# sangminwoo/Temporal-Span-Proposal-Network-VidVRD

Measured on AMD Instinct MI355X. Metric: tracklet-pairs/sec scored (N=32, T=150, D=2048), higher is better.
Workload: dtype f32

## Files before the change

include/tspn_mi355x.h:

```cpp
#ifndef TSPN_MI355X_H
#define TSPN_MI355X_H

#include <stddef.h>
#include <stdint.h>

#ifdef __cplusplus
extern "C" {
#endif

#define TSPN_ABI_VERSION 7

enum {
  TSPN_OK = 0,
  TSPN_EINVAL = -1,
  TSPN_EUNSUPPORTED = -2,
  TSPN_EWORKSPACE = -3,
  TSPN_ELAUNCH = -4,
  TSPN_EDEVICE = -5
};

#define TSPN_STATUS_WORDS 16
enum {
  TSPN_STATUS_FAULT = 0,
  TSPN_STATUS_FAULT_INFO = 1,
  TSPN_STATUS_CONV_ERR = 2,
  TSPN_STATUS_CONV_CHECKS = 3
};
enum {
  TSPN_FAULT_HANDOVER = 1
};
int tspn_status_attach(int32_t* host_words);
int tspn_status_fault(void);
int tspn_status_clear(void);
int tspn_status_selftest(int32_t* reached_end, void* stream);

#define TSPN_GEOM_CHANNELS 8

enum {
  TSPN_CONV_DIRECT = 0,
  TSPN_CONV_WINOGRAD63 = 1,
  TSPN_CONV_WINOGRAD63_F16X3 = 2
};

int tspn_version(void);
size_t tspn_fused_desc_size(void);
size_t tspn_fused_bf16_desc_size(void);
const char* tspn_last_error(void);
const char* tspn_error_string(int code);

size_t tspn_predicate_head_workspace_bytes(int64_t P, int64_t F, int64_t K);
int tspn_predicate_head_f32(const float* x, int64_t P, int64_t F, int64_t ldx,
                            const float* W, const float* b, int64_t K,
                            float* out, int apply_sigmoid,
                            void* workspace, size_t workspace_bytes, void* stream);

size_t tspn_predicate_head_norm_workspace_bytes(int64_t P, int64_t F, int64_t K, int64_t first,
                                                int64_t block, int64_t nblocks);
int tspn_predicate_head_norm_f32(const float* x, int64_t P, int64_t F, int64_t ldx,
                                 const float* W, const float* b, int64_t K,
                                 int64_t first, int64_t block, int64_t nblocks,
                                 float* out, int apply_sigmoid,
                                 void* workspace, size_t workspace_bytes, void* stream);

int tspn_feature_preprocess_f32(float* feats, int64_t P, int64_t F, int64_t ld,
                                int64_t first, int64_t block, int64_t nblocks,
                                void* stream);

int tspn_proposal_pair_filter_i64(const int64_t* pairs, const int64_t* pair_off,
                                  const int64_t* trackid, const int64_t* track_off, int64_t S,
                                  int64_t* out_idx, int64_t* out_count, int64_t* out_num_tracks,
                                  void* stream);
int tspn_gather_rows_f32(const float* src, int64_t ld, int64_t F, const int64_t* idx,
                         int64_t idx_base, int64_t R, float* out, void* stream);

int tspn_ppn_pair_matrix_topk_f32(const float* cls, int64_t B, int64_t N, int64_t Cin,
                                  int64_t H, int64_t Cout,
                                  const float* ws1, const float* bs1,
                                  const float* ws2, const float* bs2,
                                  const float* wo1, const float* bo1,
                                  const float* wo2, const float* bo2,
                                  int64_t topk, float* out_mat, int64_t* out_idx,
                                  void* stream);

int tspn_traj_iou_f32(const float* boxes1, int64_t N1, const float* boxes2, int64_t N2,
                      int64_t B, int64_t T, float* out, void* stream);

int tspn_traj_iou_tail_f64(const double* a, const int32_t* len_a, const double* b, int64_t U, int64_t N,
                           int64_t L, float* out, void* stream);

int tspn_pair_index_i64(int64_t N, int64_t base, int64_t* pairs, void* stream);

int tspn_pair_gather_f32(const float* feats, const float* boxes, int64_t NT, int64_t T,
                         int64_t D, const int64_t* pairs, int64_t P,
                         float* out_feat, float* out_geom, void* stream);

int tspn_pack_conv3_f32(const float* W, int64_t M, int64_t Cin, int64_t split,
                        float* packed, void* stream);

int tspn_conv3_f32(const float* x, int64_t B, int64_t Cin, int64_t T,
                   const float* packed, int64_t M, const float* bias, int relu,
                   float* y, void* stream);

int tspn_conv3_tc_f32(const float* x, int64_t B, int64_t T, int64_t Cin,
                      const float* packed, int64_t M, const float* bias, int relu,
                      float* y, void* stream);

int tspn_pack_conv3_wino63_frag_f32(const float* W, int64_t M, int64_t Cin, int64_t split, float* frag,
                                    void* stream);
size_t tspn_conv3_tc_wino63_workspace_bytes(int64_t B, int64_t T, int64_t Cin);
int tspn_conv3_tc_wino63_f32(const float* x, int64_t B, int64_t T, int64_t Cin, const float* frag,
                             int64_t M, const float* bias, int relu, float* y,
                             void* workspace, size_t workspace_bytes, void* stream);
int tspn_conv3_tc_wino63_set_piece_form(int form);

size_t tspn_pack_conv3_wino63_f16x3_elements(int64_t M, int64_t Cin, int64_t split);
int tspn_pack_conv3_wino63_f16x3(const float* W, int64_t M, int64_t Cin, int64_t split, int16_t* packed, void* stream);
size_t tspn_conv3_tc_wino63_f16x3_workspace_bytes(int64_t B, int64_t T, int64_t Cin, int64_t M);
int tspn_conv3_tc_wino63_f16x3(const float* x, int64_t B, int64_t T, int64_t Cin, const int16_t* packed,
                               int64_t M, const float* bias, int relu, float* y,
                               void* workspace, size_t workspace_bytes, void* stream);
int tspn_conv3_tc_wino63_f16x3_set_tail_split(int on);


int tspn_heads_f32(int mode, const float* a, const float* b, int64_t lda,
                   const int64_t* ia, const int64_t* ib, int64_t idx_stride, const float* bias,
                   const float* Wh, const float* bh, int64_t H,
                   int64_t P, int64_t C, int64_t T, float* out, void* stream);

int tspn_heads_pairgrid_f32(const float* y, int64_t B, int64_t N, int64_t C, int64_t T,
                            const float* Wh, const float* bh, int64_t H, float* out,
                            void* stream);

size_t tspn_heads_pairgrid_f16x3_split_bytes(int64_t C, int64_t H);
int tspn_heads_pairgrid_f16x3_set_force_exact(int on);
int tspn_heads_pairgrid_f16x3(const float* y, int64_t ldt, int64_t B, int64_t N, int64_t C, int64_t T,
                              const float* Wh, const float* bh, int64_t H, void* split_buf, size_t split_bytes,
                              float* out, void* stream);

int tspn_temporal_mean_f32(const float* x, int64_t R, int64_t T, int64_t Cdim,
                           int layout_tc, float* out, void* stream);
int tspn_temporal_sum_f32(const float* x, int64_t R, int64_t T, int64_t Cdim, float* out, void* stream);

int tspn_pair_rows_f32(const float* src, int64_t NT, int64_t D, const int64_t* pairs,
                       int64_t P, float* out, void* stream);

int tspn_transpose_td_f32(const float* x, int64_t R, int64_t T, int64_t D, float* out,
                          void* stream);

size_t tspn_decode_topk_workspace_bytes(int64_t S, int64_t P, int64_t topk_pair);
int tspn_decode_topk_f32(const float* rel_logit, const int64_t* pairs,
                         const float* cls_sub, const float* cls_obj, int64_t ld,
                         int64_t seg_rows, int64_t row_mul, int64_t S, int64_t P, int64_t K,
                         int64_t NO, int64_t topk_pair, int64_t topk_seg,
                         float* out_score, int64_t* out_triplet, int64_t* out_pair_tid,
                         void* workspace, size_t workspace_bytes, void* stream);

int tspn_decode_spans_f32(const float* heads, int64_t P, int64_t A, int64_t T,
                          const float* sizes_host, int64_t top_k, double nms_threshold,
                          int64_t pre_nms, int64_t* out_anchor, int64_t* out_span,
                          float* out_span_f, float* out_score, int64_t* out_count, void* stream);

typedef struct tspn_fused_desc {
  int64_t B, N, T, D;
  int64_t A, K;
  const float* feats;
  const int64_t* pairs;
  int64_t P;
  int64_t canonical_pairs;
  const float* conv_packed;
  int64_t conv_algo;
  const float* conv_bias;
  const float* head_w;
  const float* head_b;
  const float* cls_w;
  const float* cls_b;
  float* out_heads;
  float* out_logits;
  void* workspace;
  size_t workspace_bytes;
  void* ev_conv_begin;
  void* ev_conv_end;
  void* ev_logits_ready;
  const float* conv_weight;
  int64_t conv_check;
} tspn_fused_desc;

size_t tspn_forward_fused_workspace_bytes(const tspn_fused_desc* d);
int tspn_forward_fused_f32(const tspn_fused_desc* d, void* stream);

#define TSPN_CONV_CHECK_HOT_SLOTS 64
#define TSPN_CONV_CHECK_HOT_OFFSET 256
#define TSPN_CONV_CHECK_SCRATCH_BYTES (TSPN_CONV_CHECK_HOT_OFFSET + 256 * TSPN_CONV_CHECK_HOT_SLOTS)
int tspn_conv3_spot_check_f32(const float* x, int64_t B, int64_t T, int64_t Cin, const float* W, int64_t M,
                              int64_t Cw, int64_t split, const float* bias, int relu, const float* y, int64_t ldy,
                              uint64_t* scratch, int64_t rows, void* stream);

size_t tspn_span_predicate_workspace_bytes(int64_t NT, int64_t T, int64_t D, int64_t K);
int tspn_span_predicate_f32(const float* feats, int64_t NT, int64_t T, int64_t D, const int64_t* pairs,
                            const int64_t* spans, int64_t P, const float* cls_w, const float* cls_b,
                            int64_t K, float* out, void* workspace, size_t workspace_bytes, void* stream);

size_t tspn_decode_span_relations_workspace_bytes(int64_t S, int64_t N, int64_t T, int64_t D, int64_t P, int64_t J,
                                                  int64_t K, int64_t topk_per_span);
int tspn_decode_span_relations_f32(const float* feats, int64_t S, int64_t N, int64_t T, int64_t D,
                                   const int64_t* pairs, int64_t P, const int64_t* spans, const float* span_scores,
                                   const int64_t* span_counts, int64_t J, const float* cls_w, const float* cls_b,
                                   int64_t K, const float* cls_logits, int64_t NO, int64_t topk_per_span,
                                   int64_t topk_per_seg, float* out_score, int64_t* out_triplet,
                                   int64_t* out_pair_tid, int64_t* out_span, int64_t* out_span_rank,
                                   int64_t* out_valid, void* workspace, size_t workspace_bytes, void* stream);

int tspn_cast_bf16(const float* src, int64_t n, uint16_t* dst, void* stream);
int tspn_pack_conv3_bf16(const float* W, int64_t M, int64_t Cin, int64_t split, uint16_t* packed,
                         void* stream);
int tspn_pack_heads_bf16(const float* W, int64_t H, int64_t C, uint16_t* packed, void* stream);
int tspn_conv3_tc_bf16(const uint16_t* x, int64_t B, int64_t T, int64_t Cin, const uint16_t* packed,
                       int64_t M, const float* bias, float* y, int64_t ldm, void* stream);
int tspn_heads_pairgrid_bf16(const float* y, int64_t ldm, int64_t B, int64_t N, int64_t C, int64_t T,
                             const uint16_t* head_packed, const float* head_b, int64_t H, float* out,
                             void* stream);
int tspn_temporal_mean_bf16(const uint16_t* x, int64_t R, int64_t T, int64_t D, float* out, void* stream);

typedef struct tspn_fused_bf16_desc {
  int64_t B, N, T, D;
  int64_t A, K;
  const uint16_t* feats;
  const int64_t* pairs;
  int64_t P;
  const uint16_t* conv_packed;
  const float* conv_bias;
  const uint16_t* head_packed;
  const float* head_b;
  const float* cls_w;
  const float* cls_b;
  float* out_heads;
  float* out_logits;
  void* workspace;
  size_t workspace_bytes;
  void* ev_conv_begin;
  void* ev_conv_end;
  void* ev_logits_ready;
} tspn_fused_bf16_desc;

size_t tspn_forward_fused_bf16_workspace_bytes(const tspn_fused_bf16_desc* d);
int tspn_forward_fused_bf16(const tspn_fused_bf16_desc* d, void* stream);

int tspn_pair_plan_i32(const int64_t* pairs, int64_t P, int64_t B, int64_t N, int32_t* s_list, int32_t* o_list,
                       int32_t* counts, int32_t* head, int32_t* next, int32_t* rank_ws, void* stream);
size_t tspn_heads_pairlist_bf16_workspace_bytes(int64_t B, int64_t N, int64_t P);
int tspn_heads_pairlist_bf16(const float* y, int64_t ldm, int64_t B, int64_t N, int64_t C, int64_t T,
                             const int64_t* pairs, int64_t P, const uint16_t* head_packed, const float* head_b,
                             int64_t H, float* out, void* workspace, size_t workspace_bytes, void* stream);
size_t tspn_forward_fused_bf16_pairs_workspace_bytes(const tspn_fused_bf16_desc* d);
int tspn_forward_fused_bf16_pairs(const tspn_fused_bf16_desc* d, void* stream);

int tspn_pack_span_cls_bf16(const float* cls_w, int64_t K, int64_t D, uint16_t* packed, void* stream);
size_t tspn_span_predicate_bf16_workspace_bytes(int64_t NT, int64_t T, int64_t D, int64_t K, int64_t P);
int tspn_span_predicate_bf16(const uint16_t* feats, int64_t NT, int64_t T, int64_t D, const int64_t* pairs,
                             const int64_t* spans, int64_t P, const uint16_t* cls_packed, const float* cls_b,
                             int64_t K, float* out, void* workspace, size_t workspace_bytes, void* stream);
size_t tspn_decode_span_relations_bf16_workspace_bytes(int64_t S, int64_t N, int64_t T, int64_t D, int64_t P, int64_t J,
                                                       int64_t K, int64_t topk_per_span);
int tspn_decode_span_relations_bf16(const uint16_t* feats, int64_t S, int64_t N, int64_t T, int64_t D,
                                    const int64_t* pairs, int64_t P, const int64_t* spans, const float* span_scores,
                                    const int64_t* span_counts, int64_t J, const uint16_t* cls_packed,
                                    const float* cls_b, int64_t K, const float* cls_logits, int64_t NO,
                                    int64_t topk_per_span, int64_t topk_per_seg, float* out_score, int64_t* out_triplet,
                                    int64_t* out_pair_tid, int64_t* out_span, int64_t* out_span_rank,
                                    int64_t* out_valid, void* workspace, size_t workspace_bytes, void* stream);

int tspn_temporal_encoder_heads_f32(const float* x, int64_t P, int64_t C, int64_t T,
                                    const float* conv_packed, const float* conv_bias,
                                    const float* head_w, const float* head_b, int64_t H,
                                    float* h_ws, float* out_heads, void* stream);
// ... 112 lines not shown
```

temporal-span-proposal-network-vidvrd_amd/_abi.py:

```python
import ctypes
import os
import re
import threading

HERE = os.path.dirname(os.path.abspath(__file__))
ROOT = os.path.dirname(HERE)
LIB_PATH = os.environ.get("TSPN_LIB_PATH") or os.path.join(HERE, "libtspn_mi355x.so")
HEADER_PATH = os.path.join(ROOT, "include", "tspn_mi355x.h")

ABI_VERSION = 7
TSPN_OK = 0
TSPN_EINVAL = -1
TSPN_EUNSUPPORTED = -2
TSPN_EWORKSPACE = -3
TSPN_ELAUNCH = -4
TSPN_EDEVICE = -5
STATUS_WORDS = 16
STATUS_FAULT, STATUS_FAULT_INFO, STATUS_CONV_ERR, STATUS_CONV_CHECKS = 0, 1, 2, 3
FAULT_HANDOVER = 1
CONV_CHECK_HOT_OFFSET, CONV_CHECK_SCRATCH_BYTES = 256, 256 + 256 * 64
GEOM_CHANNELS = 8
CONV_DIRECT, CONV_WINOGRAD63, CONV_WINOGRAD63_F16X3 = 0, 1, 2

_c_f32p = ctypes.c_void_p
_c_i64p = ctypes.c_void_p
_i64 = ctypes.c_int64
_int = ctypes.c_int
_vp = ctypes.c_void_p
_sz = ctypes.c_size_t


class FusedDesc(ctypes.Structure):
    _fields_ = [
        ("B", _i64), ("N", _i64), ("T", _i64), ("D", _i64),
        ("A", _i64), ("K", _i64),
        ("feats", _vp), ("pairs", _vp), ("P", _i64), ("canonical_pairs", _i64),
        ("conv_packed", _vp), ("conv_algo", _i64), ("conv_bias", _vp),
        ("head_w", _vp), ("head_b", _vp),
        ("cls_w", _vp), ("cls_b", _vp),
        ("out_heads", _vp), ("out_logits", _vp),
        ("workspace", _vp), ("workspace_bytes", _sz),
        ("ev_conv_begin", _vp), ("ev_conv_end", _vp), ("ev_logits_ready", _vp),
        ("conv_weight", _vp), ("conv_check", _i64),
    ]


class FusedBf16Desc(ctypes.Structure):
    _fields_ = [
        ("B", _i64), ("N", _i64), ("T", _i64), ("D", _i64),
        ("A", _i64), ("K", _i64),
        ("feats", _vp), ("pairs", _vp), ("P", _i64),
        ("conv_packed", _vp), ("conv_bias", _vp),
        ("head_packed", _vp), ("head_b", _vp),
        ("cls_w", _vp), ("cls_b", _vp),
        ("out_heads", _vp), ("out_logits", _vp),
        ("workspace", _vp), ("workspace_bytes", _sz),
        ("ev_conv_begin", _vp), ("ev_conv_end", _vp), ("ev_logits_ready", _vp),
    ]


PROTOTYPES = {
    "tspn_version": (_int, []),
    "tspn_fused_desc_size": (_sz, []),
    "tspn_fused_bf16_desc_size": (_sz, []),
    "tspn_last_error": (ctypes.c_char_p, []),
    "tspn_error_string": (ctypes.c_char_p, [_int]),
    "tspn_status_attach": (_int, [_vp]),
    "tspn_status_fault": (_int, []),
    "tspn_status_clear": (_int, []),
    "tspn_status_selftest": (_int, [_vp, _vp]),
    "tspn_conv3_spot_check_f32": (_int, [_vp, _i64, _i64, _i64, _vp, _i64, _i64, _i64, _vp, _int, _vp, _i64, _vp, _i64, _vp]),
    "tspn_predicate_head_workspace_bytes": (_sz, [_i64, _i64, _i64]),
    "tspn_predicate_head_f32": (_int, [_vp, _i64, _i64, _i64, _vp, _vp, _i64, _vp, _int, _vp, _sz, _vp]),
    "tspn_predicate_head_norm_workspace_bytes": (_sz, [_i64, _i64, _i64, _i64, _i64, _i64]),
    "tspn_predicate_head_norm_f32": (_int, [_vp, _i64, _i64, _i64, _vp, _vp, _i64, _i64, _i64, _i64, _vp, _int,
                                            _vp, _sz, _vp]),
    "tspn_feature_preprocess_f32": (_int, [_vp, _i64, _i64, _i64, _i64, _i64, _i64, _vp]),
    "tspn_proposal_pair_filter_i64": (_int, [_vp, _vp, _vp, _vp, _i64, _vp, _vp, _vp, _vp]),
    "tspn_gather_rows_f32": (_int, [_vp, _i64, _i64, _vp, _i64, _i64, _vp, _vp]),
    "tspn_ppn_pair_matrix_topk_f32": (_int, [_vp, _i64, _i64, _i64, _i64, _i64,
                                             _vp, _vp, _vp, _vp, _vp, _vp, _vp, _vp,
                                             _i64, _vp, _vp, _vp]),
    "tspn_traj_iou_f32": (_int, [_vp, _i64, _vp, _i64, _i64, _i64, _vp, _vp]),
    "tspn_traj_iou_tail_f64": (_int, [_vp, _vp, _vp, _i64, _i64, _i64, _vp, _vp]),
    "tspn_pair_index_i64": (_int, [_i64, _i64, _vp, _vp]),
    "tspn_pair_gather_f32": (_int, [_vp, _vp, _i64, _i64, _i64, _vp, _i64, _vp, _vp, _vp]),
    "tspn_pack_conv3_f32": (_int, [_vp, _i64, _i64, _i64, _vp, _vp]),
    "tspn_conv3_f32": (_int, [_vp, _i64, _i64, _i64, _vp, _i64, _vp, _int, _vp, _vp]),
    "tspn_conv3_tc_f32": (_int, [_vp, _i64, _i64, _i64, _vp, _i64, _vp, _int, _vp, _vp]),
    "tspn_heads_f32": (_int, [_int, _vp, _vp, _i64, _vp, _vp, _i64, _vp, _vp, _vp, _i64, _i64, _i64,
                              _i64, _vp, _vp]),
    "tspn_heads_pairgrid_f32": (_int, [_vp, _i64, _i64, _i64, _i64, _vp, _vp, _i64, _vp, _vp]),
    "tspn_heads_pairgrid_f16x3_split_bytes": (_sz, [_i64, _i64]),
    "tspn_heads_pairgrid_f16x3_set_force_exact": (_int, [_int]),
    "tspn_heads_pairgrid_f16x3": (_int, [_vp, _i64, _i64, _i64, _i64, _i64, _vp, _vp, _i64, _vp, _sz, _vp, _vp]),
    "tspn_temporal_mean_f32": (_int, [_vp, _i64, _i64, _i64, _int, _vp, _vp]),
    "tspn_temporal_sum_f32": (_int, [_vp, _i64, _i64, _i64, _vp, _vp]),
    "tspn_pair_rows_f32": (_int, [_vp, _i64, _i64, _vp, _i64, _vp, _vp]),
    "tspn_transpose_td_f32": (_int, [_vp, _i64, _i64, _i64, _vp, _vp]),
    "tspn_decode_topk_workspace_bytes": (_sz, [_i64, _i64, _i64]),
    "tspn_decode_topk_f32": (_int, [_vp, _vp, _vp, _vp, _i64, _i64, _i64, _i64, _i64, _i64, _i64, _i64, _i64,
                                    _vp, _vp, _vp, _vp, _sz, _vp]),
    "tspn_decode_spans_f32": (_int, [_vp, _i64, _i64, _i64, ctypes.POINTER(ctypes.c_float), _i64,
                                     ctypes.c_double, _i64, _vp, _vp, _vp, _vp, _vp, _vp]),
    "tspn_forward_fused_workspace_bytes": (_sz, [ctypes.POINTER(FusedDesc)]),
    "tspn_forward_fused_f32": (_int, [ctypes.POINTER(FusedDesc), _vp]),
    "tspn_temporal_encoder_heads_f32": (_int, [_vp, _i64, _i64, _i64, _vp, _vp, _vp, _vp, _i64,
                                               _vp, _vp, _vp]),
    "tspn_pack_conv2d_f32": (_int, [_vp, _i64, _i64, _i64, _i64, _vp, _vp]),
    "tspn_conv2d_nhwc_f32": (_int, [_vp, _i64, _i64, _i64, _i64, _vp, _i64, _i64, _i64, _i64, _i64, _vp, _vp,
                                    _int, _vp, _vp]),
    "tspn_pack_conv2d_frag_f32": (_int, [_vp, _i64, _i64, _i64, _i64, _vp, _vp]),
    "tspn_conv2d_nhwc_frag_f32": (_int, [_vp, _i64, _i64, _i64, _i64, _vp, _i64, _i64, _i64, _i64, _i64, _vp, _vp,
                                         _int, _vp, _vp]),
    "tspn_pack_conv2d_frag_bf16": (_int, [_vp, _i64, _i64, _i64, _i64, _vp, _vp]),
    "tspn_conv2d_nhwc_bf16": (_int, [_vp, _i64, _i64, _i64, _i64, _vp, _i64, _i64, _i64, _i64, _i64, _vp, _vp,
                                     _int, _vp, _vp]),
    "tspn_roi_align_nhwc_f32": (_int, [_vp, _i64, _i64, _i64, _i64, _vp, _i64, _i64, ctypes.c_float, _int, _int,
                                       _int, _vp, _vp]),
    "tspn_pack_conv2d_frag_cin4_f32": (_int, [_vp, _i64, _i64, _i64, _i64, _vp, _vp]),
    "tspn_conv2d_nhwc_cin4_f32": (_int, [_vp, _i64, _i64, _i64, _vp, _i64, _i64, _i64, _i64, _i64, _vp, _int, _vp, _vp]),
    "tspn_max_pool_nhwc_f32": (_int, [_vp, _i64, _i64, _i64, _i64, _i64, _i64, _i64, _vp, _int, _vp]),
    "tspn_bottleneck_tail_bf16": (_int, [_vp, _i64, _i64, _i64, _i64, _vp, _vp, _vp, _vp, _vp, _vp, _vp]),
    "tspn_bottleneck_block_bf16": (_int, [_vp, _i64, _i64, _i64, _i64, _vp, _vp, _vp, _vp, _vp, _vp, _vp, _vp]),
    "tspn_bottleneck_block_proj_bf16": (_int, [_vp, _i64, _i64, _i64, _i64, _i64, _i64, _vp, _vp, _vp, _vp, _vp, _vp, _vp, _vp,
                                               _vp, _vp]),
    "tspn_bottleneck_block_res_bf16": (_int, [_vp, _i64, _i64, _i64, _i64, _i64, _i64, _vp, _vp, _vp, _vp, _vp, _vp, _vp, _vp, _vp]),
    "tspn_bottleneck_tail_io_bf16": (_int, [_vp, _i64, _i64, _i64, _i64, _vp, _vp, _vp, _vp, _vp, _vp, _vp]),
    "tspn_bottleneck_tail_pipe_bf16": (_int, [_vp, _i64, _i64, _i64, _i64, _vp, _vp, _vp, _vp, _vp, _vp, _i64, _vp]),
    "tspn_bottleneck_tail_next_bf16": (_int, [_vp, _i64, _i64, _i64, _i64, _vp, _vp, _vp, _vp, _vp, _vp, _vp, _vp, _vp, _vp]),
    "tspn_stem_bf16_workspace_bytes": (_sz, [_i64, _i64, _i64]),
    "tspn_pack_stem_bf16": (_int, [_vp, _i64, _vp, _vp]),
    "tspn_stem_conv_bf16": (_int, [_vp, _i64, _i64, _i64, _vp, _i64, _vp, _vp, _sz, _vp, _vp]),
    "tspn_max_pool_nhwc_bf16": (_int, [_vp, _i64, _i64, _i64, _i64, _i64, _i64, _i64, _vp, _vp]),
    "tspn_stem_pool_bf16": (_int, [_vp, _i64, _i64, _i64, _vp, _i64, _vp, _vp, _sz, _vp, _vp]),
    "tspn_roi_align_nhwc_bf16": (_int, [_vp, _i64, _i64, _i64, _i64, _vp, _i64, _i64, ctypes.c_float, _int, _int,
                                        _int, _vp, _vp]),
    "tspn_roi_align_nhwc_f32_bf16out": (_int, [_vp, _i64, _i64, _i64, _i64, _vp, _i64, _i64, ctypes.c_float, _int, _int,
                                               _int, _vp, _vp]),
    "tspn_pack_conv3_wino63_frag_f32": (_int, [_vp, _i64, _i64, _i64, _vp, _vp]),
    "tspn_conv3_tc_wino63_workspace_bytes": (_sz, [_i64, _i64, _i64]),
    "tspn_conv3_tc_wino63_f32": (_int, [_vp, _i64, _i64, _i64, _vp, _i64, _vp, _int, _vp, _vp, _sz, _vp]),
    "tspn_conv3_tc_wino63_set_piece_form": (_int, [_int]),
    "tspn_pack_conv3_wino63_f16x3_elements": (_sz, [_i64, _i64, _i64]),
    "tspn_pack_conv3_wino63_f16x3": (_int, [_vp, _i64, _i64, _i64, _vp, _vp]),
    "tspn_conv3_tc_wino63_f16x3_workspace_bytes": (_sz, [_i64, _i64, _i64, _i64]),
    "tspn_conv3_tc_wino63_f16x3": (_int, [_vp, _i64, _i64, _i64, _vp, _i64, _vp, _int, _vp, _vp, _sz, _vp]),
    "tspn_conv3_tc_wino63_f16x3_set_tail_split": (_int, [_int]),
    "tspn_span_predicate_workspace_bytes": (_sz, [_i64, _i64, _i64, _i64]),
    "tspn_span_predicate_f32": (_int, [_vp, _i64, _i64, _i64, _vp, _vp, _i64, _vp, _vp, _i64, _vp, _vp, _sz, _vp]),
    "tspn_decode_span_relations_workspace_bytes": (_sz, [_i64] * 8),
    "tspn_decode_span_relations_f32": (_int, [_vp, _i64, _i64, _i64, _i64, _vp, _i64, _vp, _vp, _vp, _i64, _vp, _vp, _i64,
                                              _vp, _i64, _i64, _i64, _vp, _vp, _vp, _vp, _vp, _vp, _vp, _sz, _vp]),
    "tspn_cast_bf16": (_int, [_vp, _i64, _vp, _vp]),
    "tspn_pack_conv3_bf16": (_int, [_vp, _i64, _i64, _i64, _vp, _vp]),
    "tspn_transpose_cast_bf16": (_int, [_vp, _i64, _i64, _i64, _vp, _vp]),
    "tspn_heads_dense_bf16": (_int, [_vp, _i64, _i64, _i64, _i64, _vp, _vp, _i64, _vp, _vp]),
    "tspn_temporal_encoder_heads_bf16": (_int, [_vp, _i64, _i64, _i64, _vp, _vp, _vp, _vp, _i64, _vp, _vp, _vp]),
    "tspn_pack_heads_bf16": (_int, [_vp, _i64, _i64, _vp, _vp]),
    "tspn_conv3_tc_bf16": (_int, [_vp, _i64, _i64, _i64, _vp, _i64, _vp, _vp, _i64, _vp]),
    "tspn_heads_pairgrid_bf16": (_int, [_vp, _i64, _i64, _i64, _i64, _i64, _vp, _vp, _i64, _vp, _vp]),
    "tspn_temporal_mean_bf16": (_int, [_vp, _i64, _i64, _i64, _vp, _vp]),
    "tspn_forward_fused_bf16_workspace_bytes": (_sz, [ctypes.POINTER(FusedBf16Desc)]),
    "tspn_forward_fused_bf16": (_int, [ctypes.POINTER(FusedBf16Desc), _vp]),
    "tspn_pair_plan_i32": (_int, [_vp, _i64, _i64, _i64, _vp, _vp, _vp, _vp, _vp, _vp, _vp]),
    "tspn_heads_pairlist_bf16_workspace_bytes": (_sz, [_i64, _i64, _i64]),
    "tspn_heads_pairlist_bf16": (_int, [_vp, _i64, _i64, _i64, _i64, _i64, _vp, _i64, _vp, _vp, _i64, _vp, _vp, _sz, _vp]),
    "tspn_forward_fused_bf16_pairs_workspace_bytes": (_sz, [ctypes.POINTER(FusedBf16Desc)]),
    "tspn_forward_fused_bf16_pairs": (_int, [ctypes.POINTER(FusedBf16Desc), _vp]),
    "tspn_pack_span_cls_bf16": (_int, [_vp, _i64, _i64, _vp, _vp]),
    "tspn_span_predicate_bf16_workspace_bytes": (_sz, [_i64] * 5),
    "tspn_span_predicate_bf16": (_int, [_vp, _i64, _i64, _i64, _vp, _vp, _i64, _vp, _vp, _i64, _vp, _vp, _sz, _vp]),
    "tspn_decode_span_relations_bf16_workspace_bytes": (_sz, [_i64] * 8),
    "tspn_decode_span_relations_bf16": (_int, [_vp, _i64, _i64, _i64, _i64, _vp, _i64, _vp, _vp, _vp, _i64, _vp, _vp, _i64,
                                               _vp, _i64, _i64, _i64, _vp, _vp, _vp, _vp, _vp, _vp, _vp, _sz, _vp]),
    "tspn_span_anchor_labels": (_int, [_vp, ctypes.POINTER(ctypes.c_float), _i64, _i64, _i64, _i64, ctypes.c_double,
                                      ctypes.c_double, _vp, _vp, _vp]),
    "tspn_span_loss_f32": (_int, [_vp, _vp, ctypes.POINTER(ctypes.c_float), _vp, _vp, _vp, _i64, _i64, _i64, _i64,
                                 ctypes.c_double, _vp, _vp, _vp]),
    "tspn_span_loss_finish": (_int, [_vp, _i64, _i64, _i64, _vp, _vp, _vp]),
    "tspn_span_anchor_sample_partials": (_i64, [_i64]),
    "tspn_span_anchor_sample": (_int, [_vp, _i64, ctypes.c_uint64, _int, _i64, _i64, _vp, _vp, _vp, _vp]),
    "tspn_pair_labels_f32": (_int, [_vp] * 9 + [_i64] * 6 + [ctypes.c_double, _int, _vp, _vp, _vp, _vp, _vp]),
    "tspn_eval_traj_volume_f64": (_int, [_vp, _vp, _i64, _vp, _vp]),
    "tspn_eval_viou_f64": (_int, [_vp, _vp, _vp, _vp, _vp, _i64, _vp, _vp, _vp]),
    "tspn_eval_greedy_match_f64": (_int, [_vp, _vp, _i64, _i64, ctypes.c_double, _vp, _vp, _vp, _vp]),
}

_lib = None
_lock = threading.Lock()


def header_symbols(path=HEADER_PATH):
    text = open(path).read()
    text = re.sub(r"/\*.*?\*/", "", text, flags=re.S)
    return sorted(set(re.findall(r"\b(tspn_[a-z0-9_]+)\s*\(", text)))


def lib():
    global _lib
    if _lib is not None:
        return _lib
    with _lock:
        if _lib is not None:
            return _lib
        if not os.path.exists(LIB_PATH):
            raise RuntimeError(
                f"TSPN HIP library not built: {LIB_PATH} is missing. Run "
                "`python -c 'import __graft_entry__ as g; g.build()'` (needs hipcc). "
                "There is no CPU fallback.")
        handle = ctypes.CDLL(LIB_PATH)
        for name, (res, args) in PROTOTYPES.items():
            try:
                fn = getattr(handle, name)
            except AttributeError as exc:
                raise RuntimeError(f"TSPN HIP library {LIB_PATH} does not export {name}") from exc
            fn.restype = res
            fn.argtypes = args
        if handle.tspn_version() != ABI_VERSION:
            raise RuntimeError(f"TSPN ABI version mismatch: library {LIB_PATH} reports "
                               f"{handle.tspn_version()}, host expects {ABI_VERSION} (stale build? run "
                               "__graft_entry__.build())")
        for fn, struct in (("tspn_fused_desc_size", FusedDesc), ("tspn_fused_bf16_desc_size", FusedBf16Desc)):
            if getattr(handle, fn)() != ctypes.sizeof(struct):
                raise RuntimeError(f"TSPN ABI mismatch: {fn}() = {getattr(handle, fn)()} but the host binding "
                                   f"has {ctypes.sizeof(struct)} bytes (stale {LIB_PATH}?)")
        _lib = handle
    return _lib


class TspnError(RuntimeError):
    def __init__(self, code, message):
        super().__init__(f"tspn error {code}: {message}")
        self.code = code


def check(rc):
    if rc != TSPN_OK:
        l = lib()
        msg = l.tspn_last_error().decode("utf-8", "replace")
        if not msg:
            msg = l.tspn_error_string(rc).decode()
        raise TspnError(rc, msg)
```

temporal-span-proposal-network-vidvrd_amd/build.py:

```python
import glob
import json
import os
import re
import shutil
import subprocess
import sys

HERE = os.path.dirname(os.path.abspath(__file__))
ROOT = os.path.dirname(HERE)
CSRC = os.path.join(HERE, "csrc")
CSRC_EVAL = os.path.join(CSRC, "eval")
CSRC_REL = os.path.join(CSRC, "relations")
CSRC_PAIRLIST = os.path.join(CSRC, "pairlist")
CSRC_SPANBF16 = os.path.join(CSRC, "spanbf16")
CSRC_PAIRF16 = os.path.join(CSRC, "pairf16")
CSRC_SPANLOSS = os.path.join(CSRC, "spanloss")
CSRC_SPANSAMPLE = os.path.join(CSRC, "spansample")
CSRC_PAIRLABELS = os.path.join(CSRC, "pairlabels")
LIB_NAME = "libtspn_mi355x.so"
LIB_PATH = os.path.join(HERE, LIB_NAME)
ARCH = "gfx950"

FLAGS = [
    f"--offload-arch={ARCH}", "-O3", "-std=c++17", "-fPIC",
    "-ffp-contract=off",
    "-fno-gpu-rdc", "-Wall", "-Wno-unused-function",
    "-Rpass-analysis=kernel-resource-usage",
    f"-I{os.path.join(ROOT, 'include')}", f"-I{CSRC}",
]
OBJ_DIR = os.path.join(HERE, "build", "obj")
RES_PATH = os.path.join(HERE, "kernel_resources.json")

NO_SPILL_KERNELS = ("conv3_wino63_kernel", "heads_pairgrid4_kernel", "heads_pairgrid3_kernel",
                    "conv2d_nhwc_frag_kernel", "conv2d_nhwc_bf16_kernel", "conv2d_nhwc_cin4_kernel",
                    "bottleneck_bf16_kernel", "bottleneck_pipe_bf16_kernel", "conv3_bf16_big_kernel", "heads_pairgrid_bf16_kernel",
                    "heads_pairlist_bf16_kernel", "heads_pair_f16x3_kernel",
                    "tail_io_bf16_kernel", "bottleneck_block_bf16_kernel")


def sources():
    return sorted(glob.glob(os.path.join(CSRC, "*.hip")) + glob.glob(os.path.join(CSRC_EVAL, "*.hip")) +
                  glob.glob(os.path.join(CSRC_REL, "*.hip")) + glob.glob(os.path.join(CSRC_PAIRLIST, "*.hip")) +
                  glob.glob(os.path.join(CSRC_SPANBF16, "*.hip")) + glob.glob(os.path.join(CSRC_SPANLOSS, "*.hip")) +
                  glob.glob(os.path.join(CSRC_PAIRF16, "*.hip")) + glob.glob(os.path.join(CSRC_SPANSAMPLE, "*.hip")) +
                  glob.glob(os.path.join(CSRC_PAIRLABELS, "*.hip")))


def _headers():
    return glob.glob(os.path.join(CSRC, "*.h")) + glob.glob(os.path.join(CSRC_EVAL, "*.h")) + \
        glob.glob(os.path.join(CSRC_REL, "*.h")) + glob.glob(os.path.join(CSRC_PAIRLIST, "*.h")) + \
        glob.glob(os.path.join(CSRC_SPANBF16, "*.h")) + glob.glob(os.path.join(CSRC_SPANLOSS, "*.h")) + \
        glob.glob(os.path.join(CSRC_PAIRF16, "*.h")) + glob.glob(os.path.join(CSRC_SPANSAMPLE, "*.h")) + \
        glob.glob(os.path.join(CSRC_PAIRLABELS, "*.h")) + \
        glob.glob(os.path.join(ROOT, "include", "*.h")) + \
        [os.path.abspath(__file__)]


def needs_build():
    if not os.path.exists(LIB_PATH) or not os.path.exists(RES_PATH):
        return True
    t = os.path.getmtime(LIB_PATH)
    return any(os.path.getmtime(d) > t for d in sources() + _headers())


def _obj_of(src):
    return os.path.join(OBJ_DIR, os.path.basename(src)[:-4] + ".o")


_REMARK = re.compile(r"remark:\s+(Function Name|TotalSGPRs|VGPRs|AGPRs|ScratchSize \[bytes/lane\]|Occupancy \[waves/SIMD\]|"
                     r"SGPRs Spill|VGPRs Spill|LDS Size \[bytes/block\]): (\S+)")
_KEYS = {"TotalSGPRs": "sgprs", "VGPRs": "vgprs", "AGPRs": "agprs", "ScratchSize [bytes/lane]": "scratch_bytes",
         "Occupancy [waves/SIMD]": "occupancy", "SGPRs Spill": "sgpr_spill", "VGPRs Spill": "vgpr_spill",
         "LDS Size [bytes/block]": "lds_bytes"}


def _demangle(names):
    filt = shutil.which("llvm-cxxfilt") or shutil.which("c++filt")
    if not names or not filt:
        return list(names)
    out = subprocess.run([filt], input="\n".join(names), stdout=subprocess.PIPE, text=True).stdout.split("\n")
    return out[:len(names)]


def _parse_resources(log):
    res, cur, kept, skip = {}, None, [], 0
    for line in log.split("\n"):
        m = _REMARK.search(line)
        if m:
            if m.group(1) == "Function Name":
                cur = res.setdefault(m.group(2), {})
            elif cur is not None:
                cur[_KEYS[m.group(1)]] = int(m.group(2))
            skip = 2
            continue
        if "remark:" in line and "kernel-resource-usage" in line:
            skip = 2
            continue
        if skip and (line.lstrip().startswith("|") or re.match(r"\s*\d+ \|", line)):
            skip -= 1
            continue
        skip = 0
        kept.append(line)
    names = list(res)
    return dict(zip(_demangle(names), (res[n] for n in names))), "\n".join(kept)


def _compile_one(hipcc, src, verbose):
    cmd = [hipcc] + FLAGS + ["-c", src, "-o", _obj_of(src)]
    if verbose:
        print("[tspn build]", " ".join(cmd), flush=True)
    res = subprocess.run(cmd, cwd=CSRC, stdout=subprocess.PIPE, stderr=subprocess.STDOUT, text=True)
    resources, log = _parse_resources(res.stdout)
    if res.returncode == 0:
        with open(_obj_of(src) + ".res.json", "w") as fh:
            json.dump(resources, fh, indent=1, sort_keys=True)
    return src, res.returncode, log


def kernel_resources():
    with open(RES_PATH) as fh:
        return json.load(fh)


def check_no_spill(resources):
    bad = []
    for name, r in resources.items():
        if any(k in name for k in NO_SPILL_KERNELS) and (r.get("sgpr_spill", 0) or r.get("vgpr_spill", 0)
                                                          or r.get("scratch_bytes", 0)):
            bad.append(f"{name}: {r}")
    return bad


def build(force=False, verbose=True, jobs=None):
    if not force and not needs_build():
        return LIB_PATH
    hipcc = shutil.which("hipcc") or "/opt/rocm/bin/hipcc"
    if not os.path.exists(hipcc):
        raise RuntimeError("hipcc not found: cannot build the TSPN HIP library")
    os.makedirs(OBJ_DIR, exist_ok=True)
    newest_header = max(os.path.getmtime(h) for h in _headers())
    stale = [s for s in sources()
             if force or not os.path.exists(_obj_of(s)) or not os.path.exists(_obj_of(s) + ".res.json")
             or os.path.getmtime(_obj_of(s)) < max(os.path.getmtime(s), newest_header)]
    from concurrent.futures import ThreadPoolExecutor
    jobs = jobs or min(len(stale) or 1, os.cpu_count() or 1, 8)
    with ThreadPoolExecutor(max_workers=jobs) as pool:
        results = list(pool.map(lambda s: _compile_one(hipcc, s, verbose), stale))
    for src, rc, log in results:
        if log.strip() and (verbose or rc):
            print(log, flush=True)
        if rc:
            raise RuntimeError(f"hipcc failed on {src} (exit {rc})")
    wanted = {_obj_of(s) for s in sources()}
    for o in glob.glob(os.path.join(OBJ_DIR, "*.o")):
        if o not in wanted:
            os.remove(o)
            if os.path.exists(o + ".res.json"):
                os.remove(o + ".res.json")
    resources = {}
    for o in sorted(wanted):
        with open(o + ".res.json") as fh:
            resources.update(json.load(fh))
    bad = check_no_spill(resources)
    if bad:
        raise RuntimeError("kernels with split asm load / wait sequences must not spill:\n  " + "\n  ".join(bad))
    with open(RES_PATH, "w") as fh:
        json.dump(resources, fh, indent=1, sort_keys=True)
    tmp = LIB_PATH + ".tmp"
    cmd = [hipcc, f"--offload-arch={ARCH}", "-shared", "-fPIC", "-fno-gpu-rdc"] + sorted(wanted) + ["-o", tmp]
    if verbose:
        print("[tspn build]", " ".join(cmd), flush=True)
    subprocess.run(cmd, check=True, cwd=CSRC)
    os.replace(tmp, LIB_PATH)
    return LIB_PATH


if __name__ == "__main__":
    build(force="--force" in sys.argv)
    print(LIB_PATH)
```

temporal-span-proposal-network-vidvrd_amd/csrc/pairf16/tspn_heads_pair_f16x3.hip:

```cpp
#include "tspn_common.h"
#include "tspn_device.h"

namespace {
using namespace tspn_dev;

constexpr int PF_S = 8, PF_O = 8, PF_T = 32, PF_CK = 32;
constexpr int PF_ROWS = PF_S + PF_O;
constexpr int PF_STAGE = PF_ROWS * PF_CK * PF_T;
constexpr int PF_THREADS = 64 * PF_S;
constexpr size_t PF_SMEM = sizeof(float) * 2 * PF_STAGE;
constexpr int PF_HDR_BYTES = 256;
constexpr int PF_KSTEP_BYTES = 2 * 64 * 16;
constexpr float PF_LO = 2048.f, PF_LO_INV = 1.f / 2048.f;
constexpr float PF_RANGE = 16384.f;

typedef _Float16 f16x2 __attribute__((ext_vector_type(2)));

std::atomic<int> g_force_exact{0};

__device__ __forceinline__ unsigned split_lo(unsigned h2, float as0, float as1) {
  unsigned d;
  const float neg = -PF_LO;
  asm("v_fma_mixlo_f16 %0, %1, %2, %3 op_sel_hi:[1,0,0]" : "=v"(d) : "v"(h2), "s"(neg), "v"(as0));
  asm("v_fma_mixhi_f16 %0, %1, %2, %3 op_sel:[1,0,0] op_sel_hi:[1,0,0]" : "+v"(d) : "v"(h2), "s"(neg), "v"(as1));
  return d;
}

__global__ __launch_bounds__(1024) void pairf16_scale_kernel(const float* __restrict__ Wh, int C, int H,
                                                            unsigned* __restrict__ hdr) {
  __shared__ unsigned bad_s[16];
  const int lane = threadIdx.x & 63, h = threadIdx.x >> 6;
  float mx = 0.f;
  bool finite = true;
  if (h < H) {
    for (int c = lane; c < C; c += 64) {
      const float a = fabsf(Wh[(int64_t)h * C + c]);
      finite = finite && (a < __builtin_inff());
      mx = fmaxf(mx, a);
    }
  }
#pragma unroll
  for (int o = 32; o > 0; o >>= 1) mx = fmaxf(mx, __shfl_xor(mx, o, 64));
  const bool all_finite = __all(finite);
  int e = 0;
  (void)frexpf(mx, &e);
  const bool bad = h < H && (!all_finite || !(mx >= 0x1p-100f) || e > 100);
  if (lane == 0) {
    bad_s[h] = bad ? 1u : 0u;
    hdr[1 + h] = __float_as_uint((h < H && !bad) ? ldexpf(1.f, e) : 1.f);
  }
  __syncthreads();
  if (threadIdx.x == 0) {
    unsigned f = 0;
    for (int i = 0; i < 16; ++i) f |= bad_s[i];
    hdr[0] = f;
  }
  if (threadIdx.x >= 17 && threadIdx.x < PF_HDR_BYTES / 4) hdr[threadIdx.x] = 0;
}

__global__ __launch_bounds__(64) void pairf16_pack_kernel(const float* __restrict__ Wh, int C, int H,
                                                         const unsigned* __restrict__ hdr, u32x4* __restrict__ frag) {
  const int lane = threadIdx.x, h = lane & 15, kg = lane >> 4;
  const float scale = 1.f / __uint_as_float(hdr[1 + h]);
  unsigned hi[4], lo[4];
#pragma unroll
  for (int ip = 0; ip < 4; ++ip) {
    f16x2 wh, wl;
#pragma unroll
    for (int e = 0; e < 2; ++e) {
      const int c = blockIdx.x * PF_CK + kg + 4 * (2 * ip + e);
      const float w = (h < H) ? Wh[(int64_t)h * C + c] * scale : 0.f;
      const _Float16 a = (_Float16)w;
      wh[e] = a;
      wl[e] = (_Float16)((w - (float)a) * PF_LO);
    }
    hi[ip] = __builtin_bit_cast(unsigned, wh);
    lo[ip] = __builtin_bit_cast(unsigned, wl);
  }
  frag[(int64_t)blockIdx.x * 128 + lane] = u32x4{hi[0], hi[1], hi[2], hi[3]};
  frag[(int64_t)blockIdx.x * 128 + 64 + lane] = u32x4{lo[0], lo[1], lo[2], lo[3]};
}

__device__ __noinline__ void exact_tile(const float* __restrict__ y, int64_t ldt, int C, int T, int N, int H,
                                        const float* __restrict__ Wh, const float* __restrict__ bh,
                                        float* __restrict__ out, int64_t b, int sb, int ob, int t0) {
  const int t = t0 + (threadIdx.x & 31);
  if (t >= T) return;
  for (int idx = threadIdx.x >> 5; idx < PF_S * PF_O * H; idx += PF_THREADS / 32) {
    const int pair = idx / H, h = idx - pair * H;
    const int s = sb * PF_S + (pair >> 3), o = ob * PF_O + (pair & 7);
    if (s >= N || o >= N || s == o) continue;
    const float* up = y + ((b * N + s) * 2 * (int64_t)C) * ldt + t;
    const float* vp = y + ((b * N + o) * 2 * (int64_t)C + C) * ldt + t;
    const float* w = Wh + (int64_t)h * C;
    float sum = 0.f;
    for (int c = 0; c < C; ++c) sum = __builtin_fmaf(w[c], tspn::relu_f32(up[c * ldt] + vp[c * ldt]), sum);
    const int64_t p = b * N * (int64_t)(N - 1) + (int64_t)s * (N - 1) + o - (o > s ? 1 : 0);
    out[(p * H + h) * (int64_t)T + t] = sum + (bh ? bh[h] : 0.f);
  }
}

__global__ __launch_bounds__(PF_THREADS, 1) void heads_pair_f16x3_kernel(
    const float* __restrict__ y, int64_t ldt, int C, int T, int N, int H, const float* __restrict__ Wh,
    const float* __restrict__ bh, const unsigned* __restrict__ hdr, const u32x4* __restrict__ frag,
    float* __restrict__ out, int ntb, int nob, int nsb, int64_t ngroups, int force_exact) {
  extern __shared__ __attribute__((aligned(16))) char smem_raw[];
  float* S = reinterpret_cast<float*>(smem_raw);

  const int tid = threadIdx.x;
  const int lane = tid & 63;
  const int wave = __builtin_amdgcn_readfirstlane(tid >> 6);
  const int j = lane & 15, kg = lane >> 4;
  int sb, ob;
  const int64_t G = pair_stage_group(blockIdx.x, nsb, nob, sb, ob);
  if (G >= ngroups) return;
  const int64_t b = G / ntb;
  const int t0 = (int)(G - b * ntb) * PF_T;
  const int64_t rowlen = 2 * (int64_t)C * ldt;

  if (force_exact | (int)hdr[0]) {
    exact_tile(y, ldt, C, T, N, H, Wh, bh, out, b, sb, ob, t0);
    return;
  }

  const __amdgpu_buffer_rsrc_t rsrc_y = buffer_rsrc(y + b * N * rowlen, (int)(unsigned)((int64_t)N * rowlen * 4));
  unsigned voff[2];
  const unsigned loff = (unsigned)((lane >> 3) * ldt + min((int64_t)t0 + (lane & 7) * 4, ldt - 4));
#pragma unroll
  for (int r = 0; r < 2; ++r) {
    const int row = 2 * wave + r;
    const int local = row < PF_S ? sb * PF_S + row : ob * PF_O + (row - PF_S);
    const int64_t trk = min(local, N - 1);
    voff[r] = (unsigned)((trk * rowlen + (row < PF_S ? 0 : (int64_t)C * ldt) + loff) * 4);
  }
  const int piece_bytes = (int)(8 * ldt * 4);
  int y_soff = 0;
  auto stage = [&](int buf) {
#pragma unroll
    for (int r = 0; r < 2; ++r) {
#pragma unroll
      for (int q = 0; q < 4; ++q)
        bglds16(rsrc_y, voff[r], y_soff + q * piece_bytes, S + buf * PF_STAGE + ((2 * wave + r) * PF_CK + 8 * q) * PF_T);
    }
    y_soff += 4 * piece_bytes;
  };

  f32x4 acc_hi[PF_O][2], acc_lo[PF_O][2];
#pragma unroll
  for (int o = 0; o < PF_O; ++o) {
#pragma unroll
    for (int cb = 0; cb < 2; ++cb) acc_hi[o][cb] = acc_lo[o][cb] = f32x4{0.f, 0.f, 0.f, 0.f};
  }

  const int nk = C / PF_CK;
  stage(0);
  u32x4 wh = frag[lane], wl = frag[64 + lane];
  asm volatile("s_waitcnt vmcnt(0)" ::: "memory");
  __syncthreads();
  const float* urow = S + (wave * PF_CK + kg) * PF_T + 2 * j;
  const float* vrow = S + (PF_S * PF_CK + kg) * PF_T + 2 * j;
  const float* trow = vrow + wave * PF_CK * PF_T;
  float mu = 0.f, mv = 0.f;
  for (int k = 0; k < nk; ++k) {
    const int buf = k & 1;
    u32x4 whn = wh, wln = wl;
    if (k + 1 < nk) {
      stage(buf ^ 1);
      whn = frag[(int64_t)(k + 1) * 128 + lane];
      wln = frag[(int64_t)(k + 1) * 128 + 64 + lane];
    }
    const float* ub = urow + buf * PF_STAGE;
    const float* vb = vrow + buf * PF_STAGE;
    const float* tb = trow + buf * PF_STAGE;
    f32x2 u[8];
#pragma unroll
    for (int i = 0; i < 8; ++i) {
      u[i] = *reinterpret_cast<const f32x2*>(ub + 4 * i * PF_T);
      const f32x2 vt = *reinterpret_cast<const f32x2*>(tb + 4 * i * PF_T);
      mu = __builtin_elementwise_maximum(__builtin_elementwise_maximum(mu, __builtin_fabsf(u[i][0])), __builtin_fabsf(u[i][1]));
      mv = __builtin_elementwise_maximum(__builtin_elementwise_maximum(mv, __builtin_fabsf(vt[0])), __builtin_fabsf(vt[1]));
    }
    const f16x8 a_hi = __builtin_bit_cast(f16x8, wh), a_lo = __builtin_bit_cast(f16x8, wl);
    f32x2 v[8], vn[8];
    u32x4 fh[2], fl[2], gh[2], gl[2];
#pragma unroll
    for (int i = 0; i < 8; ++i) v[i] = *reinterpret_cast<const f32x2*>(vb + 4 * i * PF_T);
#pragma unroll
    for (int o = 0; o <= PF_O; ++o) {
      if (o + 1 < PF_O) {
#pragma unroll
        for (int i = 0; i < 8; ++i) vn[i] = *reinterpret_cast<const f32x2*>(vb + ((o + 1) * PF_CK + 4 * i) * PF_T);
      }
// ... 148 lines not shown
```

temporal-span-proposal-network-vidvrd_amd/csrc/tspn_common.h:

```cpp
#pragma once
#include <hip/hip_runtime.h>

#include <atomic>
#include <cstdarg>
#include <cstdint>
#include <cstdio>
#include <initializer_list>

#include "tspn_mi355x.h"

namespace tspn {

char* err_buf();
constexpr int kErrBufLen = 512;

inline int fail(int code, const char* fmt, ...) {
  va_list ap;
  va_start(ap, fmt);
  vsnprintf(err_buf(), kErrBufLen, fmt, ap);
  va_end(ap);
  return code;
}

int status_check(const char* what);

inline int check_launch(const char* what) {
  hipError_t e = hipGetLastError();
  if (e != hipSuccess) return fail(TSPN_ELAUNCH, "%s: %s", what, hipGetErrorString(e));
  return status_check(what);
}

inline int64_t ceil_div(int64_t a, int64_t b) { return (a + b - 1) / b; }
inline bool aligned16(const void* p) { return (reinterpret_cast<uintptr_t>(p) & 15) == 0; }
template <class... P>
inline bool all_aligned16(const P*... p) {
  return (aligned16(p) && ...);
}
__host__ __device__ inline int64_t next_pow2(int64_t n) {
  int64_t p = 1;
  while (p < n) p <<= 1;
  return p;
}

__device__ __forceinline__ float relu_f32(float v) { return __builtin_elementwise_maximum(v, 0.f); }
__device__ __forceinline__ float maximum_f32(float a, float b) { return __builtin_elementwise_maximum(a, b); }

__device__ __forceinline__ unsigned order_key(float v) {
  if (v != v) return 0xffffffffu;
  const unsigned u = __float_as_uint(v + 0.f);
  return (u & 0x80000000u) ? ~u : (u | 0x80000000u);
}

__device__ __forceinline__ bool key_before(unsigned ka, int ia, unsigned kb, int ib) {
  return ka > kb || (ka == kb && ia < ib);
}

__device__ __forceinline__ unsigned long long wave_max_u64(unsigned long long v) {
#pragma unroll
  for (int o = 32; o > 0; o >>= 1) {
    const unsigned long long other = __shfl_xor(v, o, 64);
    v = other > v ? other : v;
  }
  return v;
}

struct LdsLimit {
  static constexpr int kMaxDevices = 64;
  std::atomic<size_t> set[kMaxDevices] = {};
  int ensure(const void* fn, size_t bytes, const char* what) {
    int dev = -1;
    (void)hipGetDevice(&dev);
    const bool tracked = dev >= 0 && dev < kMaxDevices;
    if (tracked && set[dev].load(std::memory_order_relaxed) >= bytes) return TSPN_OK;
    hipError_t e = hipFuncSetAttribute(fn, hipFuncAttributeMaxDynamicSharedMemorySize, (int)bytes);
    if (e != hipSuccess)
      return fail(TSPN_ELAUNCH, "%s: hipFuncSetAttribute(%zu bytes of LDS): %s", what, bytes,
                  hipGetErrorString(e));
    if (tracked) set[dev].store(bytes, std::memory_order_relaxed);
    return TSPN_OK;
  }
};

int conv3_tc_direct(const float* x, int64_t B, int64_t T, int64_t Cin, const float* packed, int64_t M,
                    const float* bias, int relu, float* y, int64_t ldy, void* stream);
bool wino63_supported(int64_t Cin, int64_t M);
size_t wino63_workspace_bytes(int64_t B, int64_t T, int64_t Cin);
int wino63_input_transform(const float* x, int64_t B, int64_t T, int64_t Cin, void* workspace,
                           size_t workspace_bytes, void* stream, uint64_t* hot = nullptr);
int wino63_contract(const void* workspace, int64_t B, int64_t T, int64_t Cin, const float* frag, int64_t M,
                    const float* bias, int relu, float* y, int64_t ldy, void* stream);
int conv3_tc_wino63(const float* x, int64_t B, int64_t T, int64_t Cin, const float* frag, int64_t M,
                    const float* bias, int relu, float* y, int64_t ldy, void* workspace,
                    size_t workspace_bytes, void* stream);
bool wino63_f16x3_supported(int64_t Cin, int64_t M);
size_t wino63_f16x3_workspace_bytes(int64_t B, int64_t T, int64_t Cin, int64_t M);
int wino63_f16x3_input_transform(const float* x, int64_t B, int64_t T, int64_t Cin, int64_t M, void* workspace,
                                 size_t workspace_bytes, void* stream, uint64_t* hot = nullptr);
int wino63_f16x3_contract(void* workspace, size_t workspace_bytes, int64_t B, int64_t T, int64_t Cin,
                          const int16_t* packed, int64_t M, const float* bias, int relu, float* y, int64_t ldy,
                          void* stream);
int heads_pairgrid(const float* y, int64_t ldt, int64_t B, int64_t N, int64_t C, int64_t T,
                   const float* Wh, const float* bh, int64_t H, float* out, void* stream, float* Wp12 = nullptr);
size_t heads_pair_f16x3_split_bytes(int64_t C, int64_t H);
bool heads_pair_f16x3_supported(const float* y, int64_t ldt, int64_t N, int64_t C, int64_t T, int64_t H, const float* out);
int heads_pair_f16x3(const float* y, int64_t ldt, int64_t B, int64_t N, int64_t C, int64_t T, const float* Wh,
                     const float* bh, int64_t H, void* split_buf, size_t split_bytes, float* out, void* stream);
inline size_t align_up(size_t a, size_t b) { return (a + b - 1) / b * b; }
int linear(const float* x, int64_t P, int64_t F, int64_t ldx, const float* W, int64_t ldw,
           const float* b, int64_t K, float* out, int apply_sigmoid, void* workspace,
           size_t workspace_bytes, void* stream);
size_t pair_predicate_workspace_bytes(int64_t NT, int64_t D, int64_t K);
int pair_predicate(const float* fbar, int64_t NT, int64_t D, const int64_t* pairs, int64_t P,
                   const float* cls_w, const float* cls_b, int64_t K, float* out, void* workspace,
                   size_t workspace_bytes, void* stream);
size_t span_prefix_workspace_bytes(int64_t NT, int64_t T, int64_t D, int64_t K);
int span_prefix_stage(const float* feats, int64_t NT, int64_t T, int64_t D, const float* cls_w, int64_t K,
                      void* workspace, size_t workspace_bytes, void* stream, const float** G_out,
                      const double** PS_out, const char* who);
inline size_t span_cand_bytes(int64_t S, int64_t P, int64_t J, int64_t R) {
  return align_up((size_t)S * P * J * R * sizeof(float), 256);
}
int segment_span_topk(const unsigned* key, const float* sc, const int* ix, const int64_t* pairs, const int64_t* spans,
                      const int64_t* span_counts, const float* cls_logits, int64_t S, int64_t N, int64_t NO, int64_t P,
                      int64_t J, int64_t R, int64_t topk_per_seg, float* out_score, int64_t* out_triplet,
                      int64_t* out_pair_tid, int64_t* out_span, int64_t* out_span_rank, int64_t* out_valid, void* stream,
                      const char* what);
int span_relation_sizes(const char* who, int64_t S, int64_t N, int64_t T, int64_t D, int64_t P, int64_t J, int64_t K,
                        int64_t NO, int64_t topk_per_span, int64_t topk_per_seg);
int span_relation_limits(const char* who, int64_t P, int64_t J, int64_t K, int64_t topk_per_span, int64_t topk_per_seg,
                         int64_t* R);

}

#define TSPN_REQUIRE(cond, code, ...)                 \
  do {                                                \
    if (!(cond)) return tspn::fail(code, __VA_ARGS__); \
  } while (0)

#define TSPN_STREAM(s) reinterpret_cast<hipStream_t>(s)

namespace tspn {

inline int tail_shape_checks(const char* what, int64_t NB, int64_t H, int64_t W, int64_t CM, bool channels_ok,
                             const char* channel_rule) {
  TSPN_REQUIRE(NB >= 0 && H > 0 && W > 0, TSPN_EINVAL, "%s: bad sizes", what);
  TSPN_REQUIRE(channels_ok, TSPN_EUNSUPPORTED, "%s: %s (got %lld)", what, channel_rule, (long long)CM);
  return TSPN_OK;
}
inline int operand_checks(const char* what, std::initializer_list<const void*> operands, bool alias_free = true,
                          const char* alias_rule = nullptr) {
  bool all = true, aligned = true;
  for (const void* p : operands) {
    all = all && p != nullptr;
    aligned = aligned && aligned16(p);
  }
  TSPN_REQUIRE(all, TSPN_EINVAL, "%s: null pointer", what);
  TSPN_REQUIRE(alias_free, TSPN_EINVAL, "%s: %s", what, alias_rule);
  TSPN_REQUIRE(aligned, TSPN_EUNSUPPORTED, "%s: operands must be 16-byte aligned", what);
  return TSPN_OK;
}
inline int tail_operand_checks(const char* what, int64_t H, int64_t W, std::initializer_list<const void*> operands) {
  if (int rc = operand_checks(what, operands)) return rc;
  TSPN_REQUIRE(H < (1 << 20) && W < (1 << 20), TSPN_EUNSUPPORTED, "%s: dimension too large", what);
  return TSPN_OK;
}

inline int window_shape_checks(const char* what, bool sizes_ok, bool window_ok, const char* window_rule, int64_t H,
                               int64_t W, int64_t KH, int64_t KW, int64_t stride, int64_t pad, int64_t* OH, int64_t* OW) {
  TSPN_REQUIRE(sizes_ok, TSPN_EINVAL, "%s: bad sizes", what);
  TSPN_REQUIRE(window_ok, TSPN_EUNSUPPORTED, "%s: %s", what, window_rule);
  TSPN_REQUIRE(H + 2 * pad >= KH && W + 2 * pad >= KW, TSPN_EINVAL, "%s: empty output", what);
  *OH = (H + 2 * pad - KH) / stride + 1, *OW = (W + 2 * pad - KW) / stride + 1;
  return TSPN_OK;
}
inline int conv_operand_checks(const char* what, const void* x, const void* w, const void* out, const void* bias,
                               const void* residual, bool channels_ok, const char* channel_rule, int64_t H, int64_t W,
                               int64_t Cin, int64_t Cout) {
  TSPN_REQUIRE(x && w && out, TSPN_EINVAL, "%s: null pointer", what);
  TSPN_REQUIRE(channels_ok, TSPN_EUNSUPPORTED, "%s: needs %s (Cin=%lld Cout=%lld)", what, channel_rule, (long long)Cin,
               (long long)Cout);
  TSPN_REQUIRE(all_aligned16(x, w, out, bias, residual), TSPN_EUNSUPPORTED, "%s: operands must be 16-byte aligned", what);
  TSPN_REQUIRE(H < (1 << 20) && W < (1 << 20) && Cin < (1 << 24) && Cout < (1 << 24), TSPN_EUNSUPPORTED,
               "%s: dimension too large", what);
  return TSPN_OK;
}

}
```

temporal-span-proposal-network-vidvrd_amd/csrc/tspn_fused.hip:

```cpp
#include <algorithm>

#include "tspn_common.h"

namespace {

struct FusedLayout {
  size_t xt, y, bias2, fbar, pooled, lin, vt, hwp, hot, psplit, total;
  size_t vt_bytes;
  size_t psplit_bytes;
  size_t lin_bytes;
};

FusedLayout layout_of(const tspn_fused_desc* d) {
  FusedLayout L{};
  const size_t NT = (size_t)d->B * d->N, T = d->T, D = d->D, C = 2 * D;
  size_t off = 0;
  auto take = [&](size_t bytes) {
    const size_t o = off;
    off += tspn::align_up(bytes, 256);
    return o;
  };
  L.xt = take(NT * D * T * sizeof(float));
  L.y = take(NT * 2 * C * tspn::align_up(T, 4) * sizeof(float));
  L.bias2 = take(2 * C * sizeof(float));
  L.fbar = take(NT * D * sizeof(float));
  L.pooled = take(256);
  L.lin_bytes = tspn::pair_predicate_workspace_bytes((int64_t)NT, (int64_t)D, d->K);
  L.lin = take(L.lin_bytes);
  L.vt_bytes = (D % 32 == 0) ? tspn::wino63_workspace_bytes((int64_t)NT, (int64_t)T, (int64_t)D) : 0;
  if (d->conv_algo == TSPN_CONV_WINOGRAD63_F16X3)
    L.vt_bytes = tspn::wino63_f16x3_workspace_bytes((int64_t)NT, (int64_t)T, (int64_t)D, (int64_t)(2 * C));
  L.vt = take(L.vt_bytes);
  L.hwp = take(C * 12 * sizeof(float));
  L.psplit_bytes = (d->conv_algo == TSPN_CONV_WINOGRAD63_F16X3 && 3 * d->A == 12)
                       ? tspn::heads_pair_f16x3_split_bytes((int64_t)C, 12) : 0;
  L.psplit = take(L.psplit_bytes);
  L.hot = take(TSPN_CONV_CHECK_SCRATCH_BYTES);
  L.total = off;
  return L;
}

int check_desc(const tspn_fused_desc* d) {
  TSPN_REQUIRE(d != nullptr, TSPN_EINVAL, "tspn_forward_fused: null descriptor");
  TSPN_REQUIRE(d->B >= 0 && d->N >= 0 && d->T > 0 && d->D > 0 && d->A > 0 && d->K > 0 &&
                   d->P >= 0,
               TSPN_EINVAL, "tspn_forward_fused: bad sizes B=%lld N=%lld T=%lld D=%lld A=%lld K=%lld P=%lld",
               (long long)d->B, (long long)d->N, (long long)d->T, (long long)d->D, (long long)d->A,
               (long long)d->K, (long long)d->P);
  TSPN_REQUIRE(3 * d->A <= 16, TSPN_EUNSUPPORTED, "tspn_forward_fused: 3*A=%lld > 16",
               (long long)(3 * d->A));
  return TSPN_OK;
}

}

extern "C" size_t tspn_forward_fused_workspace_bytes(const tspn_fused_desc* d) {
  if (check_desc(d) != TSPN_OK) return 0;
  return layout_of(d).total;
}

extern "C" int tspn_forward_fused_f32(const tspn_fused_desc* d, void* stream) {
  int rc = check_desc(d);
  if (rc) return rc;
  if (d->P == 0 || d->B * d->N == 0) return TSPN_OK;
  TSPN_REQUIRE(d->feats && d->pairs && d->conv_packed && d->conv_bias && d->head_w && d->head_b &&
                   d->cls_w && d->cls_b && d->out_heads && d->out_logits,
               TSPN_EINVAL, "tspn_forward_fused: null pointer in descriptor");
  const FusedLayout L = layout_of(d);
  TSPN_REQUIRE(d->workspace && d->workspace_bytes >= L.total, TSPN_EWORKSPACE,
               "tspn_forward_fused: workspace %zu < %zu bytes", d->workspace_bytes, L.total);
  TSPN_REQUIRE((reinterpret_cast<uintptr_t>(d->workspace) & 255) == 0, TSPN_EINVAL,
               "tspn_forward_fused: workspace must be 256-byte aligned");
  char* ws = static_cast<char*>(d->workspace);
  float* xt = reinterpret_cast<float*>(ws + L.xt);
  float* y = reinterpret_cast<float*>(ws + L.y);
  float* bias2 = reinterpret_cast<float*>(ws + L.bias2);
  float* fbar = reinterpret_cast<float*>(ws + L.fbar);
  float* pooled = reinterpret_cast<float*>(ws + L.pooled);
  void* lin = ws + L.lin;
  const int64_t NT = d->B * d->N, T = d->T, D = d->D, C = 2 * D, H = 3 * d->A;
  hipStream_t s = TSPN_STREAM(stream);

  const bool tc = (D % 16 == 0) && tspn::all_aligned16(d->feats, d->conv_packed);
  TSPN_REQUIRE(d->conv_algo == TSPN_CONV_DIRECT || d->conv_algo == TSPN_CONV_WINOGRAD63 ||
                   d->conv_algo == TSPN_CONV_WINOGRAD63_F16X3,
               TSPN_EINVAL,
               "tspn_forward_fused: conv_algo must be TSPN_CONV_DIRECT (0), TSPN_CONV_WINOGRAD63 (1) or "
               "TSPN_CONV_WINOGRAD63_F16X3 (2), got %d",
               (int)d->conv_algo);
  const bool f16x3 = d->conv_algo == TSPN_CONV_WINOGRAD63_F16X3;
  const bool w63 = d->conv_algo == TSPN_CONV_WINOGRAD63 || f16x3;
  TSPN_REQUIRE(!w63 || (tc && tspn::wino63_supported(D, 2 * C)), TSPN_EUNSUPPORTED,
               "tspn_forward_fused: TSPN_CONV_WINOGRAD63 needs D %% 32 == 0 and 16-byte aligned operands "
               "(pack the weights with tspn_pack_conv3_f32 and pass TSPN_CONV_DIRECT otherwise)");
  TSPN_REQUIRE(!f16x3 || tspn::wino63_f16x3_supported(D, 2 * C), TSPN_EUNSUPPORTED,
               "tspn_forward_fused: TSPN_CONV_WINOGRAD63_F16X3 needs D %% 64 == 0 (4D %% 256 == 0)");

  hipError_t e = hipMemsetAsync(bias2 + C, 0, C * sizeof(float), s);
  if (e == hipSuccess)
    e = hipMemcpyAsync(bias2, d->conv_bias, C * sizeof(float), hipMemcpyDeviceToDevice, s);
  if (e != hipSuccess)
    return tspn::fail(TSPN_ELAUNCH, "tspn_forward_fused: bias staging: %s", hipGetErrorString(e));

  if ((rc = tspn_temporal_mean_f32(d->feats, NT, T, D, 1, fbar, stream))) return rc;
  (void)pooled;
  if ((rc = tspn::pair_predicate(fbar, NT, D, d->pairs, d->P, d->cls_w, d->cls_b, d->K, d->out_logits, lin,
                                 L.lin_bytes, stream)))
    return rc;
  if (d->ev_logits_ready) (void)hipEventRecord(static_cast<hipEvent_t>(d->ev_logits_ready), s);

  const int64_t ldy =
      (tc && d->canonical_pairs && T % 2 == 0) ? (int64_t)tspn::align_up((size_t)T, 4) : T;
  if (!tc && (rc = tspn_transpose_td_f32(d->feats, NT, T, D, xt, stream))) return rc;
  const bool guard = w63 && d->conv_check > 0 && d->conv_weight != nullptr;
  uint64_t* hot = guard ? reinterpret_cast<uint64_t*>(ws + L.hot) : nullptr;
  if (guard && hipMemsetAsync(hot, 0, TSPN_CONV_CHECK_SCRATCH_BYTES, s) != hipSuccess)
    return tspn::fail(TSPN_ELAUNCH, "tspn_forward_fused: guard staging: %s", hipGetErrorString(hipGetLastError()));
  uint64_t* hot_slots = hot ? hot + TSPN_CONV_CHECK_HOT_OFFSET / 8 : nullptr;
  if (f16x3) {
    if ((rc = tspn::wino63_f16x3_input_transform(d->feats, NT, T, D, 2 * C, ws + L.vt, L.vt_bytes, stream, hot_slots)))
      return rc;
  } else if (w63 && (rc = tspn::wino63_input_transform(d->feats, NT, T, D, ws + L.vt, L.vt_bytes, stream, hot_slots))) {
    return rc;
  }
  if (d->ev_conv_begin) (void)hipEventRecord(static_cast<hipEvent_t>(d->ev_conv_begin), s);
  if (f16x3)
    rc = tspn::wino63_f16x3_contract(ws + L.vt, L.vt_bytes, NT, T, D, reinterpret_cast<const int16_t*>(d->conv_packed), 2 * C,
                                     bias2, 0, y, ldy, stream);
  else if (w63)
    rc = tspn::wino63_contract(ws + L.vt, NT, T, D, d->conv_packed, 2 * C, bias2, 0, y, ldy, stream);
  else
    rc = tc ? tspn::conv3_tc_direct(d->feats, NT, T, D, d->conv_packed, 2 * C, bias2, 0, y, ldy, stream)
            : tspn_conv3_f32(xt, NT, D, T, d->conv_packed, 2 * C, bias2, 0, y, stream);
  if (rc) return rc;
  if (d->ev_conv_end) (void)hipEventRecord(static_cast<hipEvent_t>(d->ev_conv_end), s);
  if (guard && (rc = tspn_conv3_spot_check_f32(d->feats, NT, T, D, d->conv_weight, C, C, D, bias2, 0, y, ldy, hot,
                                               d->conv_check, stream)))
    return rc;
  if (d->canonical_pairs) {
    TSPN_REQUIRE(d->P == d->B * d->N * (d->N - 1), TSPN_EINVAL,
                 "tspn_forward_fused: canonical_pairs needs P == B*N*(N-1) (P=%lld)", (long long)d->P);
    if (f16x3 && H == 12 && L.psplit_bytes > 0 &&
        tspn::heads_pair_f16x3_supported(y, ldy, d->N, C, T, H, d->out_heads))
      rc = tspn::heads_pair_f16x3(y, ldy, d->B, d->N, C, T, d->head_w, d->head_b, H, ws + L.psplit, L.psplit_bytes,
                                  d->out_heads, stream);
    else
      rc = tspn::heads_pairgrid(y, ldy, d->B, d->N, C, T, d->head_w, d->head_b, H, d->out_heads, stream,
                                reinterpret_cast<float*>(ws + L.hwp));
    if (rc) return rc;
  } else if ((rc = tspn_heads_f32(1, y, y + C * T, 2 * C, d->pairs, d->pairs + 1, 2, nullptr,
                                  d->head_w, d->head_b, H, d->P, C, T, d->out_heads, stream))) {
    return rc;
  }
  return TSPN_OK;
}

extern "C" int tspn_temporal_encoder_heads_f32(const float* x, int64_t P, int64_t C, int64_t T,
                                               const float* conv_packed, const float* conv_bias,
                                               const float* head_w, const float* head_b, int64_t H,
                                               float* h_ws, float* out_heads, void* stream) {
  if (P == 0) return TSPN_OK;
  TSPN_REQUIRE(x && conv_packed && head_w && h_ws && out_heads, TSPN_EINVAL,
               "tspn_temporal_encoder_heads_f32: null pointer");
  int rc = tspn_conv3_f32(x, P, C, T, conv_packed, C, conv_bias, 1, h_ws, stream);
  if (rc) return rc;
  return tspn_heads_f32(0, h_ws, nullptr, C, nullptr, nullptr, 1, nullptr, head_w, head_b, H, P, C,
                        T, out_heads, stream);
}
```

temporal-span-proposal-network-vidvrd_amd/csrc/tspn_wino63.hip:

```cpp
#include <algorithm>
#include <atomic>
#include <type_traits>

#include "tspn_common.h"
#include "tspn_device.h"

namespace {

using namespace tspn_dev;

constexpr int NW = 4;
constexpr int THREADS = 64 * NW;
constexpr int BM = 128;
constexpr int ST = 32;
constexpr int SWG = 64;
constexpr int KC = 8;
constexpr int NJ = 8;
constexpr int VROW = ST * 4;
constexpr int VCH = 2 * NJ * VROW;
constexpr int VHALF = 4 * VCH;
constexpr int VSS = 2 * VHALF;
constexpr int NVB = 2;
constexpr int NPIECE = 16;
constexpr size_t SMEM_BYTES = sizeof(float) * NVB * VSS;
#ifndef TSPN_WINO63_GM
#define TSPN_WINO63_GM 4
#endif

#ifndef TSPN_WINO63_VAUX
#define TSPN_WINO63_VAUX 0
#endif

__global__ void pack_wino63_frag_kernel(const float* __restrict__ W, int64_t M, int64_t Cin, int64_t split,
                                        float* __restrict__ out) {
  const int64_t Mp = split ? 2 * M : M, Cp = split ? split : Cin;
  const int64_t nch = Cp / KC;
  const int64_t total = NJ * Cp * Mp;
  for (int64_t o = blockIdx.x * (int64_t)blockDim.x + threadIdx.x; o < total;
       o += (int64_t)gridDim.x * blockDim.x) {
    const int e = (int)(o & 3);
    const int lane = (int)((o >> 2) & 63);
    const int64_t r = o >> 8;
    const int j = (int)(r % NJ);
    const int64_t c = (r / NJ) % nch;
    const int64_t mb = r / (NJ * nch);
    const int64_t ch = 8 * c + 4 * (lane >> 5) + e;
    const int64_t m = 32 * mb + (lane & 31);
    const float* g = (split && m >= M) ? W + ((m - M) * Cin + split + ch) * 3 : W + (m * Cin + ch) * 3;
    const double g0 = g[0], g1 = g[1], g2 = g[2];
    double u;
    switch (j) {
      case 0: u = g0; break;
      case 1: u = -2.0 / 9.0 * (g0 + g1 + g2); break;
      case 2: u = -2.0 / 9.0 * (g0 - g1 + g2); break;
      case 3: u = g0 / 90.0 + g1 / 45.0 + 2.0 * g2 / 45.0; break;
      case 4: u = g0 / 90.0 - g1 / 45.0 + 2.0 * g2 / 45.0; break;
      case 5: u = (32.0 * g0 + 16.0 * g1 + 8.0 * g2) / 45.0; break;
      case 6: u = (32.0 * g0 - 16.0 * g1 + 8.0 * g2) / 45.0; break;
      default: u = g2; break;
    }
    out[o] = (float)u;
  }
}

__device__ __forceinline__ void wino63_load_sextet(const float* __restrict__ x, int64_t b, int q, int T, int Cin,
                                                   int64_t ncols, bool ok, int channel_offset, f32x4 (&d)[8]) {
#pragma unroll
  for (int i = 0; i < 8; ++i) {
    const int t = 6 * q + i - 1;
    int64_t n = b * T + t;
    n = n < 0 ? 0 : (n < ncols ? n : ncols - 1);
    const f32x4 v = *reinterpret_cast<const f32x4*>(x + n * Cin + channel_offset);
    d[i] = (ok && t >= 0 && t < T) ? v : f32x4{0.f, 0.f, 0.f, 0.f};
  }
}
__device__ __forceinline__ void wino63_bt(const f32x4 (&d)[8], f32x4 (&V)[8]) {
  V[0] = d[0] - d[6] + 5.25f * (d[4] - d[2]);
  V[7] = d[7] - d[1] + 5.25f * (d[3] - d[5]);
  {
    const f32x4 t1 = d[2] + d[6] - 4.25f * d[4], t2 = d[1] + d[5] - 4.25f * d[3];
    V[1] = t1 + t2;
    V[2] = t1 - t2;
  }
  {
    const f32x4 t1 = d[6] + 0.25f * d[2] - 1.25f * d[4], t2 = 0.5f * d[1] - 2.5f * d[3] + 2.f * d[5];
    V[3] = t1 + t2;
    V[4] = t1 - t2;
  }
  {
    const f32x4 t1 = d[6] + 4.f * (d[2] - 1.25f * d[4]), t2 = 2.f * d[1] - 2.5f * d[3] + 0.5f * d[5];
    V[5] = t1 + t2;
    V[6] = t1 - t2;
  }
}
__device__ __forceinline__ void wino63_absmax_own_frames(const f32x4 (&d)[8], float& m) {
#pragma unroll
  for (int i = 1; i < 7; ++i)
    m = __builtin_elementwise_maximum(
        __builtin_elementwise_maximum(m, __builtin_elementwise_maximum(fabsf(d[i][0]), fabsf(d[i][1]))),
        __builtin_elementwise_maximum(fabsf(d[i][2]), fabsf(d[i][3])));
}
__device__ __forceinline__ void wino63_hot_publish(unsigned long long* __restrict__ hot, unsigned long long key, unsigned slot) {
  key = tspn::wave_max_u64(key);
  if ((threadIdx.x & 63) == 0)
    __hip_atomic_fetch_max(hot + 32 * (slot & (TSPN_CONV_CHECK_HOT_SLOTS - 1)), key, __ATOMIC_RELAXED,
                           __HIP_MEMORY_SCOPE_AGENT);
}

__global__ __launch_bounds__(256) void wino63_input_transform_kernel(
    const float* __restrict__ x, float* __restrict__ Vg, int T, int Cin, int nq, int64_t nsext, int64_t nsp,
    int64_t ncols, unsigned long long* __restrict__ hot) {
  const int lane = threadIdx.x & 63, wave = threadIdx.x >> 6;
  const int cgl = lane & 7, ql = lane >> 3;
  const int64_t S = ((int64_t)blockIdx.x * 4 + wave) * 8 + ql;
  const int cg = blockIdx.y * 8 + cgl;
  if (4 * cg >= Cin) return;
  const bool ok = S < nsext;
  const int64_t b = ok ? S / nq : 0;
  const int q = ok ? (int)(S - b * nq) : 0;
  f32x4 d[8], V[8];
  wino63_load_sextet(x, b, q, T, Cin, ncols, ok, 4 * cg, d);
  if (hot) {
    float m = 0.f;
    wino63_absmax_own_frames(d, m);
    wino63_hot_publish(hot, ((unsigned long long)__float_as_uint(m) << 32) | (unsigned)(S < nsext ? S : 0),
                       blockIdx.x * 4 + wave + 7 * blockIdx.y);
  }
  wino63_bt(d, V);
#pragma unroll
  for (int j = 0; j < 8; ++j)
    *reinterpret_cast<f32x4*>(Vg + (((int64_t)cg * NJ + j) * nsp + S) * 4) = V[j];
}

template <bool BUFV>
__global__ __launch_bounds__(THREADS) __attribute__((amdgpu_waves_per_eu(1, 1))) void conv3_wino63_kernel(
    const float* __restrict__ Vg, const float* __restrict__ Wf, const float* __restrict__ bias,
    float* __restrict__ y, int Cin, int T, int M, int nq, int64_t nsext, int64_t nsp, int tiles_m,
    int tiles_n, int relu, int ldy, int GM, int vec2) {
  extern __shared__ __attribute__((aligned(16))) char smem_raw[];
  float* Vs = reinterpret_cast<float*>(smem_raw);

  int tile_m, tile_n;
  grouped_tile(xcd_remap(blockIdx.x, gridDim.x), GM, tiles_m, tiles_n, tile_m, tile_n);
  const int m0 = tile_m * BM;
  const int64_t S0 = (int64_t)tile_n * SWG;

  const int tid = threadIdx.x;
  const int lane = tid & 63;
  const int wave = __builtin_amdgcn_readfirstlane(tid >> 6);
  const int li = lane & 31, kh = lane >> 5;
  const int nsuper = Cin >> 5;

  const char* abase;
  const unsigned aoff = lane * 16;
  {
    int mb = (m0 >> 5) + wave;
    mb = mb < (M >> 5) ? mb : 0;
    abase = reinterpret_cast<const char*>(Wf) + (int64_t)mb * (Cin / KC) * (NJ * 64 * 16);
  }

  const float* vsrc[BUFV ? 1 : NPIECE];
  unsigned voff[BUFV ? NPIECE : 1];
#pragma unroll
  for (int k = 0; k < NPIECE; ++k) {
    const int pp = NPIECE * wave + k;
    const int rr = 2 * (pp & 31) + kh;
    const int cl = rr >> 4, rem = rr & 15;
    const int g = rem >> 3, j = rem & 7;
    const int64_t e = (((int64_t)(2 * cl + g) * NJ + j) * nsp + S0 + ST * (pp >> 5) + li) * 4;
    if constexpr (BUFV) voff[k] = (unsigned)(e * 4); else vsrc[k] = Vg + e;
  }
  const int64_t super_step = (int64_t)8 * NJ * nsp * 4;
  const __amdgpu_buffer_rsrc_t rsrc_v = buffer_rsrc(Vg, (int)0xffffffffu);
  const unsigned super_bytes = (unsigned)(super_step * 4);
  auto stage_piece = [&](int S, int k) {
    if constexpr (BUFV) {
      const int soff = (int)((unsigned)S * super_bytes);
      bglds16(rsrc_v, voff[k], soff, Vs + (S & 1) * VSS + (NPIECE * wave + k) * 256);
    } else {
      glds16<TSPN_WINO63_VAUX>(vsrc[k], Vs + (S & 1) * VSS + (NPIECE * wave + k) * 256);
    }
    if constexpr (!BUFV) vsrc[k] += super_step;
  };

  f32x16 acc[2][NJ];
#pragma unroll
  for (int cb = 0; cb < 2; ++cb)
#pragma unroll
    for (int j = 0; j < NJ; ++j)
#pragma unroll
      for (int e = 0; e < 16; ++e) acc[cb][j][e] = 0.f;

  f32x4 a[2][NJ], v[2][NJ];
  const float* vlane = Vs + (kh * NJ * ST + li) * 4;
  auto load_v = [&](const float* vbuf, int cl, int j) {
    v[0][j] = *reinterpret_cast<const f32x4*>(vbuf + cl * VCH + j * VROW);
    v[1][j] = *reinterpret_cast<const f32x4*>(vbuf + VHALF + cl * VCH + j * VROW);
  };
  auto load_a_pair = [&](f32x4* ap, auto jp_tag, const char* base) {
    constexpr int JP = decltype(jp_tag)::value;
    if (JP == 0) { load_wfrag<0>(ap[0], aoff, base); load_wfrag<1024>(ap[1], aoff, base); }
    if (JP == 1) { load_wfrag<2048>(ap[2], aoff, base); load_wfrag<3072>(ap[3], aoff, base); }
    if (JP == 2) { load_wfrag<0>(ap[4], aoff, base + 4096); load_wfrag<1024>(ap[5], aoff, base + 4096); }
    if (JP == 3) { load_wfrag<2048>(ap[6], aoff, base + 4096); load_wfrag<3072>(ap[7], aoff, base + 4096); }
  };
  using P0 = std::integral_constant<int, 0>;
  using P1 = std::integral_constant<int, 1>;
  using P2 = std::integral_constant<int, 2>;
  using P3 = std::integral_constant<int, 3>;
  auto mfma_pair = [&](const f32x4* ap, int ja, int jb, int S1, int slot) {
#pragma unroll
    for (int e = 0; e < 4; ++e) {
      acc[0][ja] = __builtin_amdgcn_mfma_f32_32x32x2f32(ap[ja][e], v[0][ja][e], acc[0][ja], 0, 0, 0);
      acc[0][jb] = __builtin_amdgcn_mfma_f32_32x32x2f32(ap[jb][e], v[0][jb][e], acc[0][jb], 0, 0, 0);
      acc[1][ja] = __builtin_amdgcn_mfma_f32_32x32x2f32(ap[ja][e], v[1][ja][e], acc[1][ja], 0, 0, 0);
      if (S1 >= 0) {
        __builtin_amdgcn_sched_barrier(0);
        stage_piece(S1, 4 * slot + e);
        __builtin_amdgcn_sched_barrier(0);
      }
      acc[1][jb] = __builtin_amdgcn_mfma_f32_32x32x2f32(ap[jb][e], v[1][jb][e], acc[1][jb], 0, 0, 0);
    }
  };

#pragma unroll
  for (int k = 0; k < NPIECE; ++k) stage_piece(0, k);
  asm volatile("s_waitcnt vmcnt(0)" ::: "memory");
  __syncthreads();
#pragma unroll
  for (int j = 0; j < NJ; ++j) load_v(vlane, 0, j);
  load_a_pair(a[0], P0{}, abase); load_a_pair(a[0], P1{}, abase); load_a_pair(a[0], P2{}, abase); load_a_pair(a[0], P3{}, abase);
  abase += NJ * 1024;
  load_a_pair(a[1], P0{}, abase); load_a_pair(a[1], P1{}, abase); load_a_pair(a[1], P2{}, abase); load_a_pair(a[1], P3{}, abase);
  abase += NJ * 1024;
  __builtin_amdgcn_sched_barrier(0);

  auto chunk_body = [&](auto cl_tag, const float* vcur, const float* vnext, int S, auto has1_tag, auto has2_tag,
                        auto more_tag) {
    constexpr int CL = decltype(cl_tag)::value;
    constexpr bool HAS1 = decltype(has1_tag)::value;
    constexpr bool HAS2 = decltype(has2_tag)::value;
    constexpr bool MORE = decltype(more_tag)::value;
    constexpr int PAR = CL & 1;
    constexpr int N1 = (HAS1 ? 8 : 0) + ((MORE && CL == 1) ? NPIECE : 0);
    constexpr int N2 = (MORE && CL == 2) ? 6 : 2;
    constexpr int N0 = (HAS2 ? 2 : 0) + ((MORE && CL == 0) ? 4 : 0);
    const int S1 = (MORE && CL == 0) ? S + 1 : -1;
    const float* vn = CL == 3 ? vnext : vcur;
    constexpr int NCL = (CL + 1) & 3;
    f32x4* ap = a[PAR];
    wait_w<3 * N2 + N1>(ap[0], ap[1]);
    mfma_pair(ap, 0, 1, S1, 0);
    if (HAS2) load_a_pair(ap, P0{}, abase);
    if (HAS1) { load_v(vn, NCL, 0); load_v(vn, NCL, 1); }
    __builtin_amdgcn_sched_barrier(0);
    wait_w<2 * N2 + N1 + N0>(ap[2], ap[3]);
    mfma_pair(ap, 2, 3, S1, 1);
    if (HAS2) load_a_pair(ap, P1{}, abase);
    if (HAS1) { load_v(vn, NCL, 2); load_v(vn, NCL, 3); }
    __builtin_amdgcn_sched_barrier(0);
    wait_w<N2 + N1 + 2 * N0>(ap[4], ap[5]);
    mfma_pair(ap, 4, 5, S1, 2);
    if (HAS2) load_a_pair(ap, P2{}, abase);
    if (HAS1) { load_v(vn, NCL, 4); load_v(vn, NCL, 5); }
    __builtin_amdgcn_sched_barrier(0);
    wait_w<N1 + 3 * N0>(ap[6], ap[7]);
    mfma_pair(ap, 6, 7, S1, 3);
    if (HAS2) {
      load_a_pair(ap, P3{}, abase);
      abase += NJ * 1024;
    }
    if (HAS1) { load_v(vn, NCL, 6); load_v(vn, NCL, 7); }
    __builtin_amdgcn_sched_barrier(0);
    if (MORE && CL == 2) {
      asm volatile("s_waitcnt lgkmcnt(0)" ::: "memory");
      __builtin_amdgcn_s_barrier();
      __builtin_amdgcn_sched_barrier(0);
    }
  };
  {
    using TT = std::true_type;
    using FF = std::false_type;
    using C0 = std::integral_constant<int, 0>;
    using C1 = std::integral_constant<int, 1>;
    using C2 = std::integral_constant<int, 2>;
    using C3 = std::integral_constant<int, 3>;
    int S = 0;
    for (; S + 1 < nsuper; ++S) {
      const float* vcur = vlane + (S & 1) * VSS;
      const float* vnext = vlane + ((S + 1) & 1) * VSS;
      chunk_body(C0{}, vcur, vnext, S, TT{}, TT{}, TT{});
      chunk_body(C1{}, vcur, vnext, S, TT{}, TT{}, TT{});
      chunk_body(C2{}, vcur, vnext, S, TT{}, TT{}, TT{});
      chunk_body(C3{}, vcur, vnext, S, TT{}, TT{}, TT{});
    }
    const float* vcur = vlane + (S & 1) * VSS;
    chunk_body(C0{}, vcur, vcur, S, TT{}, TT{}, FF{});
    chunk_body(C1{}, vcur, vcur, S, TT{}, TT{}, FF{});
    chunk_body(C2{}, vcur, vcur, S, TT{}, FF{}, FF{});
    chunk_body(C3{}, vcur, vcur, S, FF{}, FF{}, FF{});
  }

#pragma unroll
  for (int cb = 0; cb < 2; ++cb) {
    const int64_t Sx = S0 + ST * cb + li;
    if (Sx < nsext) {
      const int64_t b = Sx / nq;
      const int q = (int)(Sx - b * nq);
      const int t = 6 * q;
      float* ycol = y + (b * M) * (int64_t)ldy + t;
#pragma unroll
      for (int e = 0; e < 16; ++e) {
        const int m = m0 + wave * 32 + (e & 3) + 8 * (e >> 2) + 4 * kh;
        if (m < M) {
          const float p12 = acc[cb][1][e] + acc[cb][2][e], m12 = acc[cb][1][e] - acc[cb][2][e];
          const float p34 = acc[cb][3][e] + acc[cb][4][e], m34 = acc[cb][3][e] - acc[cb][4][e];
          const float p56 = acc[cb][5][e] + acc[cb][6][e], m56 = acc[cb][5][e] - acc[cb][6][e];
          float o[6];
          o[0] = acc[cb][0][e] + p12 + p34 + p56;
          o[1] = m12 + 2.f * m34 + 0.5f * m56;
          o[2] = p12 + 4.f * p34 + 0.25f * p56;
          o[3] = m12 + 8.f * m34 + 0.125f * m56;
          o[4] = p12 + 16.f * p34 + 0.0625f * p56;
          o[5] = m12 + 32.f * m34 + 0.03125f * m56 + acc[cb][7][e];
          if (bias != nullptr) {
            const float bb = bias[m];
#pragma unroll
            for (int i = 0; i < 6; ++i) o[i] += bb;
          }
          if (relu) {
#pragma unroll
            for (int i = 0; i < 6; ++i) o[i] = tspn::relu_f32(o[i]);
          }
          float* dst = ycol + (int64_t)m * ldy;
          if (vec2) {
            *reinterpret_cast<f32x2*>(dst) = f32x2{o[0], o[1]};
            *reinterpret_cast<f32x2*>(dst + 2) = f32x2{o[2], o[3]};
            *reinterpret_cast<f32x2*>(dst + 4) = f32x2{o[4], o[5]};
          } else {
#pragma unroll
            for (int i = 0; i < 6; ++i)
              if (t + i < T) dst[i] = o[i];
          }
        }
      }
    }
  }
}

constexpr int F_BM = 256, F_BN = 256;
constexpr int F_THREADS = 512;
constexpr int F_ST = 4 * 2 * 256 * 16;
constexpr int F_NST = 4;
constexpr size_t F_SMEM = (size_t)F_NST * F_ST;
constexpr size_t F_SMEM_ALL = F_SMEM + 2 * 256 * sizeof(int);
static_assert(TSPN_WINO63_GM > 0 && TSPN_WINO63_GM < 256, "the contraction's GM argument carries the tail split and the piece form above bit 7");
constexpr size_t F_PARK_PER_TILE = (size_t)7 * F_THREADS * 128 * sizeof(float);

__device__ __forceinline__ int split_exponent(double mx) {
  if (!(mx > 0.0) || !(mx <= 1.7976931348623157e308)) return 0;
  int k;
  (void)frexp(mx, &k);
  return 15 - k;
}

__device__ __forceinline__ double wino63_u(int j, double g0, double g1, double g2) {
  switch (j) {
    case 0: return g0;
    case 1: return -2.0 / 9.0 * (g0 + g1 + g2);
    case 2: return -2.0 / 9.0 * (g0 - g1 + g2);
    case 3: return g0 / 90.0 + g1 / 45.0 + 2.0 * g2 / 45.0;
    case 4: return g0 / 90.0 - g1 / 45.0 + 2.0 * g2 / 45.0;
    case 5: return (32.0 * g0 + 16.0 * g1 + 8.0 * g2) / 45.0;
    case 6: return (32.0 * g0 - 16.0 * g1 + 8.0 * g2) / 45.0;
    default: return g2;
  }
}

__global__ void pack_wino63_frag_kernel(const float* __restrict__ W, int64_t M, int64_t Cin, int64_t split,
                                        int16_t* __restrict__ out) {
  const int64_t Mp = split ? 2 * M : M, Cp = split ? split : Cin;
  const int64_t ncg = Cp / 8;
  const int64_t o = blockIdx.x * (int64_t)blockDim.x + threadIdx.x;
  if (o >= NJ * Mp) return;
  const int j = (int)(o / Mp);
  const int64_t m = o - j * Mp;
  const float* g = (split && m >= M) ? W + ((m - M) * Cin + split) * 3 : W + (m * Cin) * 3;
  double mx = 0.0;
  for (int64_t c = 0; c < Cp; ++c) {
    const double u = fabs(wino63_u(j, g[3 * c], g[3 * c + 1], g[3 * c + 2]));
    mx = (u > mx || u != u) ? u : mx;
  }
  const int e = split_exponent(mx);
  int16_t* pj = out + (int64_t)j * (2 * ncg + 1) * Mp * 8;
  for (int64_t cg = 0; cg < ncg; ++cg) {
    f16x8 hi, lo;
#pragma unroll
    for (int i = 0; i < 8; ++i) {
      const int64_t c = 8 * cg + i;
      const double u = ldexp(wino63_u(j, g[3 * c], g[3 * c + 1], g[3 * c + 2]), e);
      const _Float16 h = (_Float16)(float)u;
      hi[i] = h;
      lo[i] = (_Float16)(float)(u - (double)(float)h);
    }
    *reinterpret_cast<f16x8*>(pj + (cg * Mp + m) * 8) = hi;
    *reinterpret_cast<f16x8*>(pj + ((ncg + cg) * Mp + m) * 8) = lo;
  }
  *reinterpret_cast<int4*>(pj + (2 * ncg * Mp + m) * 8) = int4{e, 0, 0, 0};
}

__global__ __launch_bounds__(256) void wino63_input_transform_kernel(
    const float* __restrict__ x, _Float16* __restrict__ Vh, int* __restrict__ Ve, int T, int Cin, int nq,
    int64_t nsext, int64_t nsp2, int64_t ncols, unsigned long long* __restrict__ hot) {
  __shared__ float red[4][8][NJ];
  const int tid = threadIdx.x, lane = tid & 63, wave = tid >> 6;
  const int s = tid & 7, cgs = tid >> 3;
  const int64_t S = (int64_t)blockIdx.x * 8 + s;
  const bool ok = S < nsext;
  const int64_t b = ok ? S / nq : 0;
  const int q = ok ? (int)(S - b * nq) : 0;
  const int ncg = Cin >> 3;
  auto transform = [&](int cg, f32x4 (&V)[2][8], bool want_max, float& xmax) {
#pragma unroll
    for (int h = 0; h < 2; ++h) {
      f32x4 d[8];
      wino63_load_sextet(x, b, q, T, Cin, ncols, ok, 8 * cg + 4 * h, d);
      if (want_max) wino63_absmax_own_frames(d, xmax);
      wino63_bt(d, V[h]);
    }
  };
  float cmax[NJ];
#pragma unroll
  for (int j = 0; j < NJ; ++j) cmax[j] = 0.f;
  float xm = 0.f;
  for (int cg = cgs; cg < ncg; cg += 32) {
    f32x4 V[2][8];
    transform(cg, V, hot != nullptr, xm);
#pragma unroll
    for (int j = 0; j < NJ; ++j)
#pragma unroll
      for (int h = 0; h < 2; ++h)
        cmax[j] = __builtin_elementwise_maximum(
            __builtin_elementwise_maximum(cmax[j], __builtin_elementwise_maximum(fabsf(V[h][j][0]), fabsf(V[h][j][1]))),
            __builtin_elementwise_maximum(fabsf(V[h][j][2]), fabsf(V[h][j][3])));
  }
  if (hot)
    wino63_hot_publish(hot, ((unsigned long long)__float_as_uint(xm) << 32) | (unsigned)(ok ? S : 0),
                       blockIdx.x * 4 + wave);
#pragma unroll
  for (int j = 0; j < NJ; ++j) {
    float m = cmax[j];
#pragma unroll
    for (int o = 8; o < 64; o <<= 1) m = __builtin_elementwise_maximum(m, __shfl_xor(m, o, 64));
    if (lane < 8) red[wave][lane][j] = m;
  }
  __syncthreads();
  int ecol[NJ];
#pragma unroll
  for (int j = 0; j < NJ; ++j) {
    const float m = __builtin_elementwise_maximum(__builtin_elementwise_maximum(red[0][s][j], red[1][s][j]),
                                                  __builtin_elementwise_maximum(red[2][s][j], red[3][s][j]));
    ecol[j] = split_exponent((double)m);
  }
  if (cgs == 0) {
#pragma unroll
    for (int j = 0; j < NJ; ++j) Ve[(int64_t)j * nsp2 + S] = ecol[j];
  }
  for (int cg = cgs; cg < ncg; cg += 32) {
    f32x4 V[2][8];
    transform(cg, V, false, xm);
#pragma unroll
    for (int j = 0; j < NJ; ++j) {
      f16x8 hi, lo;
#pragma unroll
      for (int i = 0; i < 8; ++i) {
        const float u = ldexpf(V[i >> 2][j][i & 3], ecol[j]);
        const _Float16 h = (_Float16)u;
        hi[i] = h;
        lo[i] = (_Float16)(u - (float)h);
      }
      _Float16* dst = Vh + (((int64_t)j * 2 * ncg + cg) * nsp2 + S) * 8;
      *reinterpret_cast<f16x8*>(dst) = hi;
      *reinterpret_cast<f16x8*>(dst + (int64_t)ncg * nsp2 * 8) = lo;
    }
  }
}

#ifndef TSPN_WINO63_F16X3_STAGGER
#define TSPN_WINO63_F16X3_STAGGER 1
#endif
template <int WN, bool BUF>
__device__ __forceinline__ void wino63_f16x3_tile(
    char* smem_raw, const _Float16* __restrict__ Vh, const int* __restrict__ Ve, const int16_t* __restrict__ Wp,
    const float* __restrict__ bias, float* __restrict__ y, float* __restrict__ park, int Cin, int T, int M, int nq,
    int64_t nsext, int64_t nsp2, int tile_m, int tile_n, int tiles_n, int sub, int relu, int ldy, int vec2) {
  constexpr int MI = WN;
  constexpr int BN = 64 * WN;
  constexpr int NP = 16 + 4 * WN;
  constexpr int PW = (NP + 7) / 8;
  constexpr bool EVEN = NP % 8 == 0;
  constexpr bool STAGGER = TSPN_WINO63_F16X3_STAGGER && WN == 4;
  const int m0 = tile_m * F_BM;
  const int64_t S0 = (int64_t)tile_n * F_BN + sub * BN;

  const int tid = threadIdx.x;
  const int lane = tid & 63;
  const int wave = __builtin_amdgcn_readfirstlane(tid >> 6);
  const int wm = wave / WN, wn = wave % WN;
  const int li = lane & 31, kh = lane >> 5;
  const int ncg = Cin >> 3, nk = Cin >> 4;
  const int G = NJ * nk;

  const int p0 = wave * NP / 8;
  const int npw = EVEN ? PW : (wave + 1) * NP / 8 - p0;
  const int16_t* src[PW];
  unsigned voff[PW];
  int ldst[PW];
#pragma unroll
  for (int i = 0; i < PW; ++i) {
    const int p = min(p0 + i, NP - 1);
    int64_t el;
    if (p < 16) {
      const int region = p >> 3, cgi = (p >> 2) & 1, r = 64 * (p & 3) + lane;
      el = (((int64_t)region * ncg + cgi) * M + m0 + r) * 8;
      src[i] = Wp + el;
      ldst[i] = p * 1024;
    } else {
      const int v = p - 16;
      const int region = v / (2 * WN), cgi = (v / WN) & 1, r = 64 * (v % WN) + lane;
      el = (((int64_t)region * ncg + cgi) * nsp2 + S0 + r) * 8;
      src[i] = reinterpret_cast<const int16_t*>(Vh) + el;
      ldst[i] = (2 + region) * 8192 + cgi * 4096 + (v % WN) * 1024;
    }
    voff[i] = (unsigned)(el * 2);
  }
  int ik = 0, ist = 0;
  const char* wbase = reinterpret_cast<const char*>(Wp);
  const char* vbase = reinterpret_cast<const char*>(Vh);
  auto issue = [&]() {
    char* dst = smem_raw + ist * F_ST;
#pragma unroll
    for (int i = 0; i < PW; ++i)
      if (EVEN || i < npw) {
        if (BUF) bglds16(buffer_rsrc_unbounded(p0 + i < 16 ? wbase : vbase), voff[i], 0, dst + ldst[i]);
        else glds16(src[i], dst + ldst[i]);
      }
    ist = (ist + 1) & 3;
    const bool wrap = ++ik == nk;
    if (wrap) ik = 0;
    const int64_t dw = (int64_t)M * (wrap ? 32 * nk + 48 : 32), dv = nsp2 * (wrap ? 32 * nk + 32 : 32);
    if (BUF) {
      wbase += dw;
      vbase += dv;
    } else {
#pragma unroll
      for (int i = 0; i < PW; ++i) src[i] = reinterpret_cast<const int16_t*>(reinterpret_cast<const char*>(src[i]) + (p0 + i < 16 ? dw : dv));
    }
  };
  auto wait_stages = [&](auto ahead_tag) {
    constexpr int AHEAD = decltype(ahead_tag)::value;
    if (EVEN || npw == PW) wait_vmcnt<AHEAD * PW>(); else wait_vmcnt<AHEAD * (PW - 1)>();
  };

  f32x16 acc[MI][2];
#pragma unroll
  for (int mi = 0; mi < MI; ++mi)
#pragma unroll
    for (int ni = 0; ni < 2; ++ni)
#pragma unroll
      for (int e = 0; e < 16; ++e) acc[mi][ni][e] = 0.f;

  float* my_park = park + (int64_t)(tile_m * tiles_n + tile_n) * (F_PARK_PER_TILE / sizeof(float)) +
                   (int64_t)sub * (8 * MI) * F_THREADS * 4 + tid * 4;
  int* etab = reinterpret_cast<int*>(smem_raw + F_SMEM);
  auto unscale = [&](int j) {
    if (tid < F_BM)
      etab[tid] = reinterpret_cast<const int*>(Wp + (int64_t)j * (2 * ncg + 1) * M * 8 + (int64_t)2 * ncg * M * 8)[(int64_t)(m0 + tid) * 4];
    else if (tid - F_BM < BN)
      etab[tid] = Ve[(int64_t)j * nsp2 + S0 + tid - F_BM];
    __syncthreads();
    int ec[2];
#pragma unroll
    for (int ni = 0; ni < 2; ++ni) ec[ni] = etab[F_BM + wn * 64 + ni * 32 + li];
#pragma unroll
    for (int mi = 0; mi < MI; ++mi)
#pragma unroll
      for (int e = 0; e < 16; ++e) {
        const int r = etab[wm * (32 * MI) + mi * 32 + (e & 3) + 8 * (e >> 2) + 4 * kh];
#pragma unroll
        for (int ni = 0; ni < 2; ++ni) acc[mi][ni][e] = ldexpf(acc[mi][ni][e], -(r + ec[ni]));
      }
  };

  f16x8 ah[MI], al[MI], bh[2][2], bl[2];
  const int a_off = (kh * 256 + wm * (32 * MI) + li) * 16, b_off = (kh * 256 + wn * 64 + li) * 16;
  auto read_hi = [&](int st, f16x8 (&bhn)[2]) {
    const char* s = smem_raw + st * F_ST;
#pragma unroll
    for (int mi = 0; mi < MI; ++mi) ah[mi] = *reinterpret_cast<const f16x8*>(s + a_off + mi * 512);
#pragma unroll
    for (int ni = 0; ni < 2; ++ni) bhn[ni] = *reinterpret_cast<const f16x8*>(s + 16384 + b_off + ni * 512);
  };
  auto read_lo = [&](int st) {
    const char* s = smem_raw + st * F_ST;
#pragma unroll
    for (int ni = 0; ni < 2; ++ni) bl[ni] = *reinterpret_cast<const f16x8*>(s + 24576 + b_off + ni * 512);
#pragma unroll
    for (int mi = 0; mi < MI; ++mi) al[mi] = *reinterpret_cast<const f16x8*>(s + 8192 + a_off + mi * 512);
  };
  auto group = [&](const f16x8 (&a)[MI], const f16x8 (&b)[2]) {
#pragma unroll
    for (int ni = 0; ni < 2; ++ni)
#pragma unroll
      for (int mi = 0; mi < MI; ++mi) acc[mi][ni] = __builtin_amdgcn_mfma_f32_32x32x16_f16(a[mi], b[ni], acc[mi][ni], 0, 0, 0);
  };
  auto point_end = [&](int j) {
    unscale(j);
    if (j < NJ - 1) {
#pragma unroll
      for (int mi = 0; mi < MI; ++mi)
#pragma unroll
        for (int ni = 0; ni < 2; ++ni)
#pragma unroll
          for (int eq = 0; eq < 4; ++eq) {
            const f32x4 v = {acc[mi][ni][4 * eq], acc[mi][ni][4 * eq + 1], acc[mi][ni][4 * eq + 2], acc[mi][ni][4 * eq + 3]};
            *reinterpret_cast<f32x4*>(my_park + ((int64_t)j * 32 + (mi * 2 + ni) * 4 + eq) * F_THREADS * 4) = v;
#pragma unroll
            for (int e = 0; e < 4; ++e) acc[mi][ni][4 * eq + e] = 0.f;
          }
    }
    __builtin_amdgcn_sched_barrier(0);
  };
// ... 150 lines not shown
  L.e = tspn::align_up((size_t)NJ * 2 * Cin * nsp2 * sizeof(_Float16), 256);
  L.park = L.e + tspn::align_up((size_t)NJ * nsp2 * sizeof(int), 256);
  L.total = L.park + (size_t)tspn::ceil_div(M, F_BM) * (nsp2 / F_BN) * F_PARK_PER_TILE;
  return L;
}

int check_common(const char* what, int64_t B, int64_t T, int64_t Cin, int64_t M, int64_t ldy) {
  TSPN_REQUIRE(B >= 0 && Cin > 0 && T > 0 && M > 0 && ldy >= T && ldy < (1 << 24), TSPN_EINVAL,
               "%s: bad sizes B=%lld T=%lld Cin=%lld M=%lld ldy=%lld", what, (long long)B, (long long)T,
               (long long)Cin, (long long)M, (long long)ldy);
  TSPN_REQUIRE(tspn::wino63_supported(Cin, M), TSPN_EUNSUPPORTED,
               "%s: needs Cin %% 32 == 0, M %% 32 == 0 (Cin=%lld M=%lld)", what, (long long)Cin, (long long)M);
  TSPN_REQUIRE(Cin < (1 << 24) && T < (1 << 24) && M < (1 << 24), TSPN_EUNSUPPORTED, "%s: dimension too large", what);
  return TSPN_OK;
}

}

bool tspn::wino63_supported(int64_t Cin, int64_t M) { return Cin > 0 && M > 0 && Cin % 32 == 0 && M % 32 == 0; }

size_t tspn::wino63_workspace_bytes(int64_t B, int64_t T, int64_t Cin) {
  if (B <= 0 || T <= 0 || Cin <= 0 || Cin % 32 != 0) return 0;
  return (size_t)(Cin / 4) * NJ * (size_t)padded_sextets(B, T) * 4 * sizeof(float);
}

extern "C" size_t tspn_conv3_tc_wino63_workspace_bytes(int64_t B, int64_t T, int64_t Cin) {
  return tspn::wino63_workspace_bytes(B, T, Cin);
}

extern "C" int tspn_pack_conv3_wino63_frag_f32(const float* W, int64_t M, int64_t Cin, int64_t split, float* frag,
                                               void* stream) {
  TSPN_REQUIRE(W && frag, TSPN_EINVAL, "tspn_pack_conv3_wino63_frag_f32: null pointer");
  TSPN_REQUIRE(M > 0 && Cin > 0 && split >= 0, TSPN_EINVAL, "tspn_pack_conv3_wino63_frag_f32: bad sizes");
  TSPN_REQUIRE(split == 0 || Cin == 2 * split, TSPN_EINVAL,
               "tspn_pack_conv3_wino63_frag_f32: split=%lld requires Cin == 2*split (Cin=%lld)", (long long)split,
               (long long)Cin);
  const int64_t Mp = split ? 2 * M : M, Cp = split ? split : Cin;
  TSPN_REQUIRE(Cp % KC == 0 && Mp % 32 == 0, TSPN_EUNSUPPORTED,
               "tspn_pack_conv3_wino63_frag_f32: needs (packed) Cin %% 8 == 0 and M %% 32 == 0 (Cin=%lld M=%lld)",
               (long long)Cp, (long long)Mp);
  const int64_t total = NJ * Cp * Mp;
  const int blocks = (int)std::min<int64_t>(tspn::ceil_div(total, 256), 8192);
  hipLaunchKernelGGL(pack_wino63_frag_kernel, dim3(blocks), dim3(256), 0, TSPN_STREAM(stream), W, M, Cin, split, frag);
  return tspn::check_launch("tspn_pack_conv3_wino63_frag_f32");
}

int tspn::wino63_input_transform(const float* x, int64_t B, int64_t T, int64_t Cin, void* workspace,
                                 size_t workspace_bytes, void* stream, uint64_t* hot) {
  const char* what = "tspn_conv3_tc_wino63_f32(input transform)";
  if (int rc = check_common(what, B, T, Cin, 32, T)) return rc;
  if (B == 0) return TSPN_OK;
  TSPN_REQUIRE(x && tspn::aligned16(x), TSPN_EINVAL, "%s: x must be a 16-byte aligned pointer", what);
  const size_t need = tspn::wino63_workspace_bytes(B, T, Cin);
  TSPN_REQUIRE(workspace && workspace_bytes >= need, TSPN_EWORKSPACE, "%s: workspace %zu < %zu bytes", what,
               workspace_bytes, need);
  TSPN_REQUIRE(tspn::aligned16(workspace), TSPN_EINVAL, "%s: workspace must be 16-byte aligned",
               what);
  const int64_t nq = tspn::ceil_div(T, 6);
  const int64_t nsext = B * nq, nsp = padded_sextets(B, T);
  TSPN_REQUIRE(nsp / 32 < (1LL << 31) && Cin / 32 < 65536, TSPN_EUNSUPPORTED, "%s: grid too large", what);
  hipLaunchKernelGGL(wino63_input_transform_kernel, dim3((unsigned)(nsp / 32), (unsigned)(Cin / 32)), dim3(256), 0,
                     TSPN_STREAM(stream), x, static_cast<float*>(workspace), (int)T, (int)Cin, (int)nq, nsext, nsp,
                     B * T, reinterpret_cast<unsigned long long*>(hot));
  return tspn::check_launch(what);
}

static std::atomic<int> g_piece_form{0};

int tspn::wino63_contract(const void* workspace, int64_t B, int64_t T, int64_t Cin, const float* frag, int64_t M,
                          const float* bias, int relu, float* y, int64_t ldy, void* stream) {
  const char* what = "tspn_conv3_tc_wino63_f32";
  if (int rc = check_common(what, B, T, Cin, M, ldy)) return rc;
  if (B == 0) return TSPN_OK;
  TSPN_REQUIRE(workspace && frag && y, TSPN_EINVAL, "%s: null pointer", what);
  TSPN_REQUIRE(tspn::aligned16(frag) && (reinterpret_cast<uintptr_t>(y) & 3) == 0,
               TSPN_EUNSUPPORTED, "%s: frag must be 16-byte aligned", what);
  const int64_t nq = tspn::ceil_div(T, 6);
  const int64_t nsext = B * nq, nsp = padded_sextets(B, T);
  const int64_t tiles_m = tspn::ceil_div(M, BM), tiles_n = nsp / SWG;
  TSPN_REQUIRE(tiles_m * tiles_n < (1LL << 31), TSPN_EUNSUPPORTED, "%s: grid too large", what);
  const int vec2 = (ldy % 2 == 0) && (ldy >= 6 * nq) && ((reinterpret_cast<uintptr_t>(y) & 7) == 0);
#ifndef TSPN_WINO63_BUFV
#define TSPN_WINO63_BUFV 1
#endif
  const bool bufv = TSPN_WINO63_BUFV && tspn::wino63_workspace_bytes(B, T, Cin) < (1ull << 32) &&
                    g_piece_form.load(std::memory_order_relaxed) == 0;
  static tspn::LdsLimit lds[2];
  auto launch = [&](auto kern, tspn::LdsLimit& lim) {
    if (int rc = lim.ensure(reinterpret_cast<const void*>(kern), SMEM_BYTES, what)) return rc;
    hipLaunchKernelGGL(kern, dim3((unsigned)(tiles_m * tiles_n)), dim3(THREADS), SMEM_BYTES, TSPN_STREAM(stream),
                       static_cast<const float*>(workspace), frag, bias, y, (int)Cin, (int)T, (int)M, (int)nq, nsext, nsp,
                       (int)tiles_m, (int)tiles_n, relu, (int)ldy, TSPN_WINO63_GM, vec2);
    return tspn::check_launch(what);
  };
  return bufv ? launch(conv3_wino63_kernel<true>, lds[1]) : launch(conv3_wino63_kernel<false>, lds[0]);
}

int tspn::conv3_tc_wino63(const float* x, int64_t B, int64_t T, int64_t Cin, const float* frag, int64_t M,
                          const float* bias, int relu, float* y, int64_t ldy, void* workspace,
                          size_t workspace_bytes, void* stream) {
  if (int rc = check_common("tspn_conv3_tc_wino63_f32", B, T, Cin, M, ldy)) return rc;
  if (int rc = tspn::wino63_input_transform(x, B, T, Cin, workspace, workspace_bytes, stream)) return rc;
  return tspn::wino63_contract(workspace, B, T, Cin, frag, M, bias, relu, y, ldy, stream);
}

extern "C" int tspn_conv3_tc_wino63_set_piece_form(int form) {
  TSPN_REQUIRE(form == 0 || form == 1, TSPN_EINVAL, "tspn_conv3_tc_wino63_set_piece_form: form must be 0 or 1");
  return g_piece_form.exchange(form, std::memory_order_relaxed);
}

extern "C" int tspn_conv3_tc_wino63_f32(const float* x, int64_t B, int64_t T, int64_t Cin, const float* frag,
                                        int64_t M, const float* bias, int relu, float* y, void* workspace,
                                        size_t workspace_bytes, void* stream) {
  return tspn::conv3_tc_wino63(x, B, T, Cin, frag, M, bias, relu, y, T, workspace, workspace_bytes, stream);
}

bool tspn::wino63_f16x3_supported(int64_t Cin, int64_t M) {
  return Cin > 0 && M > 0 && Cin % 32 == 0 && M % F_BM == 0 && Cin < (1 << 24) && M < (1 << 24);
}

size_t tspn::wino63_f16x3_workspace_bytes(int64_t B, int64_t T, int64_t Cin, int64_t M) {
  if (B <= 0 || T <= 0 || !tspn::wino63_f16x3_supported(Cin, M)) return 0;
  return f16x3_layout(B, T, Cin, M).total;
}

extern "C" size_t tspn_conv3_tc_wino63_f16x3_workspace_bytes(int64_t B, int64_t T, int64_t Cin, int64_t M) {
  return tspn::wino63_f16x3_workspace_bytes(B, T, Cin, M);
}

extern "C" size_t tspn_pack_conv3_wino63_f16x3_elements(int64_t M, int64_t Cin, int64_t split) {
  if (M <= 0 || Cin <= 0 || split < 0 || (split && Cin != 2 * split)) return 0;
  const int64_t Mp = split ? 2 * M : M, Cp = split ? split : Cin;
  return (size_t)NJ * (2 * (Cp / 8) + 1) * Mp * 8;
}

extern "C" int tspn_pack_conv3_wino63_f16x3(const float* W, int64_t M, int64_t Cin, int64_t split, int16_t* packed,
                                            void* stream) {
  const char* what = "tspn_pack_conv3_wino63_f16x3";
  TSPN_REQUIRE(W && packed, TSPN_EINVAL, "%s: null pointer", what);
  TSPN_REQUIRE(M > 0 && Cin > 0 && split >= 0, TSPN_EINVAL, "%s: bad sizes", what);
  TSPN_REQUIRE(split == 0 || Cin == 2 * split, TSPN_EINVAL, "%s: split=%lld requires Cin == 2*split (Cin=%lld)", what,
               (long long)split, (long long)Cin);
  TSPN_REQUIRE(tspn::aligned16(packed), TSPN_EINVAL, "%s: packed must be 16-byte aligned", what);
  const int64_t Mp = split ? 2 * M : M, Cp = split ? split : Cin;
  TSPN_REQUIRE(tspn::wino63_f16x3_supported(Cp, Mp), TSPN_EUNSUPPORTED,
               "%s: needs (packed) Cin %% 32 == 0 and M %% 256 == 0 (Cin=%lld M=%lld)", what, (long long)Cp, (long long)Mp);
  void (*kern)(const float*, int64_t, int64_t, int64_t, int16_t*) = pack_wino63_frag_kernel;
  hipLaunchKernelGGL(kern, dim3((unsigned)tspn::ceil_div(NJ * Mp, 256)), dim3(256), 0, TSPN_STREAM(stream), W, M, Cin,
                     split, packed);
  return tspn::check_launch(what);
}

int tspn::wino63_f16x3_input_transform(const float* x, int64_t B, int64_t T, int64_t Cin, int64_t M, void* workspace,
                                       size_t workspace_bytes, void* stream, uint64_t* hot) {
  const char* what = "tspn_conv3_tc_wino63_f16x3(input transform)";
  if (int rc = check_common(what, B, T, Cin, 32, T)) return rc;
  TSPN_REQUIRE(tspn::wino63_f16x3_supported(Cin, M), TSPN_EUNSUPPORTED,
               "%s: needs Cin %% 32 == 0 and M %% 256 == 0 (Cin=%lld M=%lld)", what, (long long)Cin, (long long)M);
  if (B == 0) return TSPN_OK;
  TSPN_REQUIRE(x && tspn::aligned16(x), TSPN_EINVAL, "%s: x must be a 16-byte aligned pointer", what);
  const F16x3Layout L = f16x3_layout(B, T, Cin, M);
  TSPN_REQUIRE(workspace && workspace_bytes >= L.total, TSPN_EWORKSPACE, "%s: workspace %zu < %zu bytes", what,
               workspace_bytes, L.total);
  TSPN_REQUIRE((reinterpret_cast<uintptr_t>(workspace) & 255) == 0, TSPN_EINVAL, "%s: workspace must be 256-byte aligned",
               what);
  const int64_t nq = tspn::ceil_div(T, 6);
  const int64_t nsext = B * nq, nsp2 = padded_sextets_f16x3(B, T);
  TSPN_REQUIRE(nsp2 / 8 < (1LL << 31), TSPN_EUNSUPPORTED, "%s: grid too large", what);
  char* ws = static_cast<char*>(workspace);
  void (*kern)(const float*, _Float16*, int*, int, int, int, int64_t, int64_t, int64_t, unsigned long long*) =
      wino63_input_transform_kernel;
  hipLaunchKernelGGL(kern, dim3((unsigned)(nsp2 / 8)), dim3(256), 0, TSPN_STREAM(stream), x,
                     reinterpret_cast<_Float16*>(ws + L.v), reinterpret_cast<int*>(ws + L.e), (int)T, (int)Cin, (int)nq,
                     nsext, nsp2, B * T, reinterpret_cast<unsigned long long*>(hot));
  return tspn::check_launch(what);
}

static std::atomic<int> g_tail_split{1};

extern "C" int tspn_conv3_tc_wino63_f16x3_set_tail_split(int on) {
  TSPN_REQUIRE(on == 0 || on == 1, TSPN_EINVAL, "tspn_conv3_tc_wino63_f16x3_set_tail_split: on must be 0 or 1");
  return g_tail_split.exchange(on, std::memory_order_relaxed);
}

static int device_cus() {
  constexpr int kMaxDevices = 64;
  static std::atomic<int> cached[kMaxDevices] = {};
  int dev = -1, cus = 0;
  if (hipGetDevice(&dev) != hipSuccess) return 0;
  const bool tracked = dev >= 0 && dev < kMaxDevices;
  if (tracked && (cus = cached[dev].load(std::memory_order_relaxed)) > 0) return cus;
  if (hipDeviceGetAttribute(&cus, hipDeviceAttributeMultiprocessorCount, dev) != hipSuccess || cus <= 0) return 0;
  if (tracked) cached[dev].store(cus, std::memory_order_relaxed);
  return cus;
}

static int tail_split_factor(int64_t tiles, int cus, int64_t* R) {
  *R = 0;
  if (cus <= 0 || g_tail_split.load(std::memory_order_relaxed) == 0) return 1;
  const int64_t r = tiles % cus;
  if (r == 0) return 1;
  const int64_t f = std::min<int64_t>(4, cus / r);
  if (f < 2) return 1;
  *R = r;
  return f == 3 ? 2 : (int)f;
}

int tspn::wino63_f16x3_contract(void* workspace, size_t workspace_bytes, int64_t B, int64_t T, int64_t Cin,
                                const int16_t* packed, int64_t M, const float* bias, int relu, float* y, int64_t ldy,
                                void* stream) {
  const char* what = "tspn_conv3_tc_wino63_f16x3";
  if (int rc = check_common(what, B, T, Cin, M, ldy)) return rc;
  TSPN_REQUIRE(tspn::wino63_f16x3_supported(Cin, M), TSPN_EUNSUPPORTED,
               "%s: needs Cin %% 32 == 0 and M %% 256 == 0 (Cin=%lld M=%lld)", what, (long long)Cin, (long long)M);
  if (B == 0) return TSPN_OK;
  TSPN_REQUIRE(workspace && packed && y, TSPN_EINVAL, "%s: null pointer", what);
  TSPN_REQUIRE(tspn::aligned16(packed) && (reinterpret_cast<uintptr_t>(y) & 3) == 0,
               TSPN_EUNSUPPORTED, "%s: packed weights must be 16-byte aligned", what);
  const F16x3Layout L = f16x3_layout(B, T, Cin, M);
  TSPN_REQUIRE(workspace_bytes >= L.total, TSPN_EWORKSPACE, "%s: workspace %zu < %zu bytes", what, workspace_bytes,
               L.total);
  const int64_t nq = tspn::ceil_div(T, 6);
  const int64_t nsext = B * nq, nsp2 = padded_sextets_f16x3(B, T);
  const int64_t tiles_m = M / F_BM, tiles_n = nsp2 / F_BN;
  TSPN_REQUIRE(tiles_m * tiles_n < (1LL << 29), TSPN_EUNSUPPORTED, "%s: grid too large", what);
  const int vec2 = (ldy % 2 == 0) && (ldy >= 6 * nq) && ((reinterpret_cast<uintptr_t>(y) & 7) == 0);
  int64_t R = 0;
  const int f = tail_split_factor(tiles_m * tiles_n, device_cus(), &R);
  const int64_t grid = tiles_m * tiles_n + R * (f - 1);
  const int64_t slab = 4 * Cin * std::max<int64_t>(M, nsp2);
  const int buf = slab < (1LL << 31) && g_piece_form.load(std::memory_order_relaxed) == 0;
  char* ws = static_cast<char*>(workspace);
  static tspn::LdsLimit lds;
  void (*kern)(const _Float16*, const int*, const int16_t*, const float*, float*, float*, int, int, int, int, int64_t,
               int64_t, int, int, int, int, int, int) = conv3_wino63_kernel;
  if (int rc = lds.ensure(reinterpret_cast<const void*>(kern), F_SMEM_ALL, what)) return rc;
  hipLaunchKernelGGL(kern, dim3((unsigned)grid), dim3(F_THREADS), F_SMEM_ALL, TSPN_STREAM(stream),
                     reinterpret_cast<const _Float16*>(ws + L.v), reinterpret_cast<const int*>(ws + L.e), packed, bias, y,
                     reinterpret_cast<float*>(ws + L.park), (int)Cin, (int)T, (int)M, (int)nq, nsext, nsp2, (int)tiles_m,
                     (int)tiles_n, relu, (int)ldy, TSPN_WINO63_GM | (f << 8) | (buf << 16), vec2);
  return tspn::check_launch(what);
}

extern "C" int tspn_conv3_tc_wino63_f16x3(const float* x, int64_t B, int64_t T, int64_t Cin, const int16_t* packed,
                                          int64_t M, const float* bias, int relu, float* y, void* workspace,
                                          size_t workspace_bytes, void* stream) {
  const char* what = "tspn_conv3_tc_wino63_f16x3";
  if (int rc = check_common(what, B, T, Cin, M, T)) return rc;
  TSPN_REQUIRE(tspn::wino63_f16x3_supported(Cin, M), TSPN_EUNSUPPORTED,
               "%s: needs Cin %% 32 == 0 and M %% 256 == 0 (Cin=%lld M=%lld)", what, (long long)Cin, (long long)M);
  if (B > 0) {
    TSPN_REQUIRE(workspace && packed && y, TSPN_EINVAL, "%s: null pointer", what);
    TSPN_REQUIRE(tspn::aligned16(packed) && (reinterpret_cast<uintptr_t>(y) & 3) == 0,
                 TSPN_EUNSUPPORTED, "%s: packed weights must be 16-byte aligned", what);
  }
  if (int rc = tspn::wino63_f16x3_input_transform(x, B, T, Cin, M, workspace, workspace_bytes, stream)) return rc;
  return tspn::wino63_f16x3_contract(workspace, workspace_bytes, B, T, Cin, packed, M, bias, relu, y, T, stream);
}
```

temporal-span-proposal-network-vidvrd_amd/ops.py:

```python
import ctypes
import threading

import torch

from . import _abi

__all__ = [
    "predicate_head", "feature_preprocess_", "ppn_pair_matrix_topk", "traj_iou", "traj_iou_tail", "pair_index",
    "pair_gather", "pack_conv3", "conv3", "conv3_tc", "pack_conv3_wino63", "conv3_tc_wino63", "pack_conv3_wino63_f16x3", "conv3_tc_wino63_f16x3", "heads", "heads_pairgrid", "heads_pairgrid_f16x3", "heads_pairgrid_f16x3_split_bytes",
    "heads_pairgrid_f16x3_set_force_exact", "temporal_mean", "temporal_sum", "pair_rows", "transpose_td",
    "forward_fused", "temporal_encoder_heads", "fused_workspace_bytes", "fused_bf16_workspace_bytes", "decode_topk", "decode_spans", "decode_span_relations",
    "span_anchor_labels", "span_loss", "span_anchor_sample", "pair_labels",
    "cast_bf16", "pack_conv3_bf16", "pack_heads_bf16", "conv3_tc_bf16", "heads_pairgrid_bf16",
    "pair_plan", "heads_pairlist_bf16",
    "transpose_cast_bf16", "temporal_encoder_heads_bf16",
    "temporal_mean_bf16", "forward_fused_bf16", "span_predicate",
    "pack_span_cls_bf16", "span_predicate_bf16", "decode_span_relations_bf16", "bottleneck_block_bf16", "bottleneck_block_proj_bf16", "bottleneck_block_res_bf16",
    "proposal_pair_filter", "gather_rows", "wino63_set_piece_form", "wino63_f16x3_set_tail_split", "conv3_spot_check",
    "pack_conv2d", "pack_conv2d_frag", "conv2d_nhwc", "roi_align_nhwc", "pack_conv2d_frag_bf16", "conv2d_nhwc_bf16", "max_pool_nhwc", "pack_conv2d_frag_cin4", "conv2d_nhwc_cin4", "max_pool_nhwc_bf16", "pack_stem_bf16", "stem_conv_bf16", "stem_pool_bf16", "bottleneck_tail_bf16",
    "eval_traj_volume", "eval_viou", "eval_greedy_match",
    "status_words", "status_fault", "status_clear", "status_selftest",
]


_status_blocks = {}
_status_lock = threading.Lock()


def _status_block(index=None):
    idx = torch.cuda.current_device() if index is None else int(index)
    blk = _status_blocks.get(idx)
    if blk is not None:
        return blk
    with _status_lock:
        blk = _status_blocks.get(idx)
        if blk is None:
            raw = torch.zeros(_abi.STATUS_WORDS + 16, dtype=torch.int32).pin_memory()
            off = (-(raw.data_ptr() // 4)) % 16
            blk = raw[off:off + _abi.STATUS_WORDS]
            with torch.cuda.device(idx):
                _abi.check(_abi.lib().tspn_status_attach(ctypes.c_void_p(blk.data_ptr())))
            blk = _status_blocks[idx] = blk.numpy()
    return blk


def _stream():
    blk = _status_block()
    fault = int(blk[_abi.STATUS_FAULT])
    if fault:
        raise _abi.TspnError(_abi.TSPN_EDEVICE,
                             f"device {torch.cuda.current_device()} reported fault 0x{fault:x}"
                             + (" (an LDS hand-over between waves timed out)" if fault & _abi.FAULT_HANDOVER else "")
                             + f", info 0x{int(blk[_abi.STATUS_FAULT_INFO]) & 0xffffffff:x}, in an earlier launch of this library: "
                             "results produced since are not to be trusted; ops.status_clear() re-arms")
    return ctypes.c_void_p(torch.cuda.current_stream().cuda_stream)


def status_words(device=None):
    return _status_block(None if device is None else torch.device(device).index)


def status_fault(device=None):
    return int(status_words(device)[_abi.STATUS_FAULT])


def status_clear(device=None):
    w = status_words(device)
    w[_abi.STATUS_FAULT_INFO] = 0
    w[_abi.STATUS_FAULT] = 0


def status_selftest(device=None):
    dev = torch.device("cuda", torch.cuda.current_device()) if device is None else torch.device(device)
    with torch.cuda.device(dev):
        reached = torch.zeros(1, dtype=torch.int32, device=dev)
        _status_block()
        _abi.check(_abi.lib().tspn_status_selftest(_p(reached), ctypes.c_void_p(torch.cuda.current_stream().cuda_stream)))
    return reached


def _first_hip_device(obj, depth=0):
    if isinstance(obj, torch.Tensor):
        return obj.device if obj.is_cuda else None
    if depth < 2:
        if isinstance(obj, (list, tuple)):
            for v in obj:
                d = _first_hip_device(v, depth + 1)
                if d is not None:
                    return d
        elif isinstance(obj, dict):
            for v in obj.values():
                d = _first_hip_device(v, depth + 1)
                if d is not None:
                    return d
    return None


def _on_tensor_device(fn):
    import functools

    @functools.wraps(fn)
    def wrapper(*args, **kwargs):
        dev = None
        for a in list(args) + list(kwargs.values()):
            d = _first_hip_device(a)
            if d is None:
                continue
            if dev is None:
                dev = d
            elif d != dev:
                raise RuntimeError(f"{fn.__name__}: operands live on different devices ({dev} and {d})")
        if dev is None or dev.index == torch.cuda.current_device():
            return fn(*args, **kwargs)
        with torch.cuda.device(dev):
            return fn(*args, **kwargs)
    return wrapper


def _dev(t, name, dtype=torch.float32):
    if not isinstance(t, torch.Tensor):
        raise TypeError(f"{name}: expected a torch.Tensor, got {type(t).__name__}")
    if not t.is_cuda:
        raise RuntimeError(f"{name}: tensor is on {t.device}; the TSPN HIP path needs a HIP device "
                           "tensor (there is no CPU fallback)")
    if t.dtype != dtype:
        raise TypeError(f"{name}: expected {dtype}, got {t.dtype}")
    if not t.is_contiguous():
        raise ValueError(f"{name}: tensor must be contiguous")
    return t


def _p(t):
    return ctypes.c_void_p(t.data_ptr()) if t is not None else ctypes.c_void_p(0)


def _ws(nbytes, device):
    return torch.empty(max(int(nbytes), 256), dtype=torch.uint8, device=device)


def _workspace(workspace, need, device, who, sizes=False):
    if workspace is None:
        return _ws(need, device)
    if workspace.numel() * workspace.element_size() < need:
        raise ValueError(f"{who}: workspace too small" + (f" ({workspace.numel()} < {need})" if sizes else ""))
    return workspace


def _toggle(setter, value):
    prev = getattr(_abi.lib(), setter)(int(value))
    if prev < 0:
        _abi.check(prev)
    return prev


def _out_hw(who, H, W, KH, KW, stride, padding):
    OH, OW = (H + 2 * padding - KH) // stride + 1, (W + 2 * padding - KW) // stride + 1
    if OH <= 0 or OW <= 0:
        raise ValueError(f"{who}: empty output")
    return OH, OW


def predicate_head(x, weight, bias, apply_sigmoid=True, norm=None):
    _dev(x, "x"); _dev(weight, "weight")
    if bias is not None:
        _dev(bias, "bias")
    if x.dim() != 2 or weight.dim() != 2 or x.shape[1] != weight.shape[1]:
        raise ValueError(f"predicate_head: shapes {tuple(x.shape)} x {tuple(weight.shape)}^T do not match")
    if bias is not None and bias.shape != (weight.shape[0],):
        raise ValueError("predicate_head: bias shape mismatch")
    P, F = x.shape
    K = weight.shape[0]
# ... 145 lines not shown
    if want_feat:
        _dev(tracklet_feats, "tracklet_feats")
        NT, T, D = tracklet_feats.shape
        feat = torch.empty((P, 2 * D, T), dtype=torch.float32, device=pairs.device)
    if want_geom:
        _dev(tracklet_boxes, "tracklet_boxes")
        if tracklet_boxes.dim() != 3 or tracklet_boxes.shape[2] != 4:
            raise ValueError("pair_gather: tracklet_boxes must be [N,T,4]")
        if NT is not None and tuple(tracklet_boxes.shape[:2]) != (NT, T):
            raise ValueError("pair_gather: feats / boxes shape mismatch")
        NT, T = tracklet_boxes.shape[:2]
        if out_geom is None:
            geom = torch.empty((P, _abi.GEOM_CHANNELS, T), dtype=torch.float32, device=pairs.device)
        else:
            _dev(out_geom, "out_geom")
            if tuple(out_geom.shape) != (P, _abi.GEOM_CHANNELS, T):
                raise ValueError(f"pair_gather: out_geom must be [{P},{_abi.GEOM_CHANNELS},{T}], got {tuple(out_geom.shape)}")
            geom = out_geom
        D = D or 1
    if NT is None:
        return None, None
    if check_pairs and P and (int(pairs.min()) < 0 or int(pairs.max()) >= NT):
        raise IndexError("pair_gather: pair index out of range")
    _abi.check(_abi.lib().tspn_pair_gather_f32(
        _p(tracklet_feats if want_feat else None), _p(tracklet_boxes if want_geom else None),
        NT, T, D, _p(pairs), P, _p(feat), _p(geom), _stream()))
    return feat, geom


def pack_conv3(weight, split=0):
    _dev(weight, "conv weight")
    if weight.dim() != 3 or weight.shape[2] != 3:
        raise ValueError("pack_conv3: weight must be [M,Cin,3]")
    M, Cin, _ = weight.shape
    if split:
        shape = (3, split, 2 * M)
    else:
        shape = (3, Cin, M)
    packed = torch.empty(shape, dtype=torch.float32, device=weight.device)
    _abi.check(_abi.lib().tspn_pack_conv3_f32(_p(weight), M, Cin, split, _p(packed), _stream()))
    return packed


def conv3(x, packed, bias=None, relu=False):
    _dev(x, "x"); _dev(packed, "packed")
    if bias is not None:
        _dev(bias, "bias")
    B, Cin, T = x.shape
    if packed.dim() != 3 or packed.shape[0] != 3 or packed.shape[1] != Cin:
        raise ValueError(f"conv3: packed weights {tuple(packed.shape)} do not match Cin={Cin}")
    M = packed.shape[2]
    if bias is not None and bias.shape != (M,):
        raise ValueError("conv3: bias shape mismatch")
    y = torch.empty((B, M, T), dtype=torch.float32, device=x.device)
    _abi.check(_abi.lib().tspn_conv3_f32(_p(x), B, Cin, T, _p(packed), M, _p(bias), 1 if relu else 0,
                                         _p(y), _stream()))
    return y


def conv3_tc(x, packed, bias=None, relu=False):
    _dev(x, "x"); _dev(packed, "packed")
    if bias is not None:
        _dev(bias, "bias")
    B, T, Cin = x.shape
    if packed.dim() != 3 or packed.shape[0] != 3 or packed.shape[1] != Cin:
        raise ValueError(f"conv3_tc: packed weights {tuple(packed.shape)} do not match Cin={Cin}")
    M = packed.shape[2]
    y = torch.empty((B, M, T), dtype=torch.float32, device=x.device)
    _abi.check(_abi.lib().tspn_conv3_tc_f32(_p(x), B, T, Cin, _p(packed), M, _p(bias), 1 if relu else 0,
                                            _p(y), _stream()))
    return y


def wino63_frag_dims(frag):
    if frag.dim() != 5 or tuple(frag.shape[2:]) != (8, 64, 4):
        raise ValueError(f"not a fragment-major F(6,3) weight tensor: {tuple(frag.shape)}")
    return frag.shape[1] * 8, frag.shape[0] * 32


def pack_conv3_wino63(weight, split=0):
    _dev(weight, "conv weight")
    if weight.dim() != 3 or weight.shape[2] != 3:
        raise ValueError("pack_conv3_wino63: weight must be [M,Cin,3]")
    M, Cin, _ = weight.shape
    Mp, Cp = (2 * M, split) if split else (M, Cin)
    if Cp % 8 or Mp % 32:
        raise ValueError(f"pack_conv3_wino63: needs Cin % 8 == 0 and M % 32 == 0 (Cin={Cp}, M={Mp})")
    frag = torch.empty((Mp // 32, Cp // 8, 8, 64, 4), dtype=torch.float32, device=weight.device)
    _abi.check(_abi.lib().tspn_pack_conv3_wino63_frag_f32(_p(weight), M, Cin, split, _p(frag), _stream()))
    return frag


def conv3_tc_wino63(x, frag, bias=None, relu=False, workspace=None):
    _dev(x, "x"); _dev(frag, "frag")
    if bias is not None:
        _dev(bias, "bias")
    B, T, Cin = x.shape
    cin_w, M = wino63_frag_dims(frag)
    if cin_w != Cin:
        raise ValueError(f"conv3_tc_wino63: weights are for Cin={cin_w}, x has Cin={Cin}")
    l = _abi.lib()
    need = l.tspn_conv3_tc_wino63_workspace_bytes(B, T, Cin)
    workspace = _workspace(workspace, need, x.device, "conv3_tc_wino63", sizes=True)
    y = torch.empty((B, M, T), dtype=torch.float32, device=x.device)
    _abi.check(l.tspn_conv3_tc_wino63_f32(_p(x), B, T, Cin, _p(frag), M, _p(bias), 1 if relu else 0, _p(y),
                                          _p(workspace), workspace.numel() * workspace.element_size(), _stream()))
    return y


def wino63_f16x3_dims(packed):
    if packed.dim() != 4 or packed.dtype != torch.int16 or packed.shape[0] != 8 or packed.shape[3] != 8 \
            or packed.shape[1] % 2 != 1:
        raise ValueError(f"not a split-fp16 F(6,3) weight tensor: {tuple(packed.shape)} {packed.dtype}")
    return (packed.shape[1] - 1) // 2 * 8, packed.shape[2]


def pack_conv3_wino63_f16x3(weight, split=0):
    _dev(weight, "conv weight")
    if weight.dim() != 3 or weight.shape[2] != 3:
        raise ValueError("pack_conv3_wino63_f16x3: weight must be [M,Cin,3]")
    M, Cin, _ = weight.shape
    Mp, Cp = (2 * M, split) if split else (M, Cin)
    if Cp % 32 or Mp % 256:
        raise ValueError(f"pack_conv3_wino63_f16x3: needs Cin % 32 == 0 and M % 256 == 0 (Cin={Cp}, M={Mp})")
    packed = torch.empty((8, 2 * (Cp // 8) + 1, Mp, 8), dtype=torch.int16, device=weight.device)
    assert packed.numel() == _abi.lib().tspn_pack_conv3_wino63_f16x3_elements(M, Cin, split)
    _abi.check(_abi.lib().tspn_pack_conv3_wino63_f16x3(_p(weight), M, Cin, split, _p(packed), _stream()))
    return packed


def conv3_tc_wino63_f16x3(x, packed, bias=None, relu=False, workspace=None):
    _dev(x, "x")
    if bias is not None:
        _dev(bias, "bias")
    B, T, Cin = x.shape
    cin_w, M = wino63_f16x3_dims(packed)
    if cin_w != Cin:
        raise ValueError(f"conv3_tc_wino63_f16x3: weights are for Cin={cin_w}, x has Cin={Cin}")
    l = _abi.lib()
    need = l.tspn_conv3_tc_wino63_f16x3_workspace_bytes(B, T, Cin, M)
    workspace = _workspace(workspace, need, x.device, "conv3_tc_wino63_f16x3", sizes=True)
    y = torch.empty((B, M, T), dtype=torch.float32, device=x.device)
    _abi.check(l.tspn_conv3_tc_wino63_f16x3(_p(x), B, T, Cin, _p(packed), M, _p(bias), 1 if relu else 0, _p(y),
                                            _p(workspace), workspace.numel() * workspace.element_size(), _stream()))
    return y


def wino63_set_piece_form(form):
    return _toggle("tspn_conv3_tc_wino63_set_piece_form", form)


def wino63_f16x3_set_tail_split(on):
    return _toggle("tspn_conv3_tc_wino63_f16x3_set_tail_split", on)


def heads(a, head_w, head_b, b=None, ia=None, ib=None, bias=None, channels=None, num_pairs=None):
    _dev(a, "a"); _dev(head_w, "head_w")
    mode = 0 if b is None else 1
    lda, T = a.shape[1], a.shape[2]
    C = channels if channels is not None else lda
    H = head_w.shape[0]
    if head_w.shape[1] != C:
        raise ValueError("heads: head_w / channel mismatch")
    for nm, t in (("ia", ia), ("ib", ib)):
        if t is not None:
            _dev(t, nm, torch.int64)
    if b is not None:
        _dev(b, "b")
        if b.shape[1:] != a.shape[1:]:
            raise ValueError("heads: a / b shape mismatch")
    if num_pairs is None:
        num_pairs = ia.shape[0] if ia is not None else a.shape[0]
    out = torch.empty((num_pairs, H, T), dtype=torch.float32, device=a.device)
    _abi.check(_abi.lib().tspn_heads_f32(mode, _p(a), _p(b), lda, _p(ia), _p(ib), 1, _p(bias),
                                         _p(head_w), _p(head_b), H, num_pairs, C, T, _p(out), _stream()))
    return out


def heads_pairgrid(y, B, N, head_w, head_b):
    _dev(y, "y"); _dev(head_w, "head_w")
    NT, C2, T = y.shape
    C, H = C2 // 2, head_w.shape[0]
    if NT != B * N or head_w.shape[1] != C:
        raise ValueError("heads_pairgrid: shape mismatch")
    out = torch.empty((B * N * max(N - 1, 0), H, T), dtype=torch.float32, device=y.device)
    _abi.check(_abi.lib().tspn_heads_pairgrid_f32(_p(y), B, N, C, T, _p(head_w), _p(head_b), H, _p(out),
                                                  _stream()))
    return out


def heads_pairgrid_f16x3_split_bytes(C, H):
    return int(_abi.lib().tspn_heads_pairgrid_f16x3_split_bytes(int(C), int(H)))


def heads_pairgrid_f16x3_set_force_exact(on):
    return _toggle("tspn_heads_pairgrid_f16x3_set_force_exact", on)


def heads_pairgrid_f16x3(y, B, N, head_w, head_b, T=None, split_buf=None, out=None):
    _dev(y, "y"); _dev(head_w, "head_w")
    NT, C2, ldt = y.shape
    T = ldt if T is None else int(T)
    C, H = C2 // 2, head_w.shape[0]
    if NT != B * N or head_w.shape[1] != C:
        raise ValueError("heads_pairgrid_f16x3: shape mismatch")
    if split_buf is None:
        split_buf = _ws(heads_pairgrid_f16x3_split_bytes(C, H), y.device)
    if out is None:
        out = torch.empty((B * N * max(N - 1, 0), H, T), dtype=torch.float32, device=y.device)
    _abi.check(_abi.lib().tspn_heads_pairgrid_f16x3(_p(y), ldt, B, N, C, T, _p(head_w), _p(head_b), H, _p(split_buf),
                                                    split_buf.numel(), _p(out), _stream()))
    return out


def temporal_mean(x, layout_tc):
    _dev(x, "x")
    if layout_tc:
        R, T, Cd = x.shape
    else:
        R, Cd, T = x.shape
    out = torch.empty((R, Cd), dtype=torch.float32, device=x.device)
    _abi.check(_abi.lib().tspn_temporal_mean_f32(_p(x), R, T, Cd, 1 if layout_tc else 0, _p(out), _stream()))
    return out


def temporal_sum(x):
    _dev(x, "x")
    R, T, Cd = x.shape
    out = torch.empty((R, Cd), dtype=torch.float32, device=x.device)
    _abi.check(_abi.lib().tspn_temporal_sum_f32(_p(x), R, T, Cd, _p(out), _stream()))
    return out


def pair_rows(src, pairs):
    _dev(src, "src"); _dev(pairs, "pairs", torch.int64)
    NT, D = src.shape
    P = pairs.shape[0]
    out = torch.empty((P, 2 * D), dtype=torch.float32, device=src.device)
    _abi.check(_abi.lib().tspn_pair_rows_f32(_p(src), NT, D, _p(pairs), P, _p(out), _stream()))
    return out


def transpose_td(x):
    _dev(x, "x")
    R, T, D = x.shape
    out = torch.empty((R, D, T), dtype=torch.float32, device=x.device)
    _abi.check(_abi.lib().tspn_transpose_td_f32(_p(x), R, T, D, _p(out), _stream()))
    return out


def decode_topk(rel_logit, pairs, cls_sub, cls_obj=None, row_mul=1, num_obj=35,
                topk_per_pair=20, topk_per_seg=200, check_pairs=True):
    squeeze = rel_logit.dim() == 2
    if squeeze:
        rel_logit, pairs, cls_sub = rel_logit.unsqueeze(0), pairs.unsqueeze(0), cls_sub.unsqueeze(0)
        cls_obj = cls_obj.unsqueeze(0) if cls_obj is not None else None
    _dev(rel_logit, "rel_logit"); _dev(pairs, "pairs", torch.int64); _dev(cls_sub, "cls_sub")
    S, P, K = rel_logit.shape
    if tuple(pairs.shape) != (S, P, 2):
        raise ValueError("decode_topk: pairs must be [S,P,2]")
    if cls_sub.dim() != 3 or cls_sub.shape[0] != S:
        raise ValueError("decode_topk: class logits must be [S,rows,cols]")
    seg_rows, ld = cls_sub.shape[1], cls_sub.shape[2]
    if cls_obj is None:
        if ld >= 2 * num_obj:
            obj_ptr = cls_sub.data_ptr() + 4 * num_obj
        else:
            obj_ptr = cls_sub.data_ptr()
    else:
        _dev(cls_obj, "cls_obj")
        if cls_obj.shape != cls_sub.shape:
            raise ValueError("decode_topk: cls_obj shape mismatch")
        obj_ptr = cls_obj.data_ptr()
    if check_pairs and P and (int(pairs.min()) < 0 or int(pairs.max()) * row_mul >= seg_rows):
        raise IndexError("decode_topk: row_mul * tracklet id exceeds the class-logit rows")
    R = min(topk_per_pair, K)
    M = min(topk_per_seg, P * R)
    dev = rel_logit.device
    scores = torch.empty((S, M), dtype=torch.float32, device=dev)
    trip = torch.empty((S, M, 3), dtype=torch.int64, device=dev)
    tids = torch.empty((S, M, 2), dtype=torch.int64, device=dev)
    l = _abi.lib()
    ws = _ws(l.tspn_decode_topk_workspace_bytes(S, P, R), dev)
    _abi.check(l.tspn_decode_topk_f32(_p(rel_logit), _p(pairs), _p(cls_sub), ctypes.c_void_p(obj_ptr), ld,
                                      seg_rows, row_mul, S, P, K, num_obj, topk_per_pair, topk_per_seg,
                                      _p(scores), _p(trip), _p(tids), _p(ws), ws.numel(), _stream()))
    return (scores[0], trip[0], tids[0]) if squeeze else (scores, trip, tids)


def decode_spans(heads, sizes, top_k=64, nms_threshold=0.5, pre_nms=1024):
    _dev(heads, "heads")
    P, H, T = heads.shape
    A = len(sizes)
    if H != 3 * A:
        raise ValueError(f"decode_spans: heads has {H} channels, expected 3*A = {3 * A}")
    dev = heads.device
    out = {"anchor": torch.empty((P, top_k), dtype=torch.int64, device=dev),
           "span": torch.empty((P, top_k, 2), dtype=torch.int64, device=dev),
           "span_f": torch.empty((P, top_k, 2), dtype=torch.float32, device=dev),
           "score": torch.empty((P, top_k), dtype=torch.float32, device=dev),
           "count": torch.empty((P,), dtype=torch.int64, device=dev)}
    sz = (ctypes.c_float * A)(*[float(v) for v in sizes])
    _abi.check(_abi.lib().tspn_decode_spans_f32(_p(heads), P, A, T, sz, top_k, float(nms_threshold), pre_nms,
                                                _p(out["anchor"]), _p(out["span"]), _p(out["span_f"]),
                                                _p(out["score"]), _p(out["count"]), _stream()))
    return out
# ... 965 lines not shown
```

Measured before the change: 1.251 million.

## Fuse temporal mean and exponent scan into a streaming f16x3 Winograd input pass

Adds a per-tracklet scan kernel that streams frames once to compute the temporal mean, per-sextet Winograd exponents, and the conv-check hot keys together, followed by a separate split kernel that writes the hi/lo f16 planes. In the fused forward, this replaces the standalone temporal-mean kernel and the monolithic input transform when Cin >= 1024 and there are enough tracklets per CU. The goal is to avoid reading the feature tensor separately for the mean and for the exponent pass. It keeps two launches, and the split kernel still rereads x. A smaller change vectorizes the head-weight absmax scan with float4 loads.

```diff
diff --git a/include/tspn_mi355x.h b/include/tspn_mi355x.h
--- a/include/tspn_mi355x.h
+++ b/include/tspn_mi355x.h
@@ -120,6 +120,10 @@
                                int64_t M, const float* bias, int relu, float* y,
                                void* workspace, size_t workspace_bytes, void* stream);
 int tspn_conv3_tc_wino63_f16x3_set_tail_split(int on);
+int tspn_conv3_tc_wino63_f16x3_input_form(int64_t NT, int64_t T, int64_t Cin, int cus);
+int tspn_conv3_tc_wino63_f16x3_set_input_form(int form);
+int tspn_conv3_tc_wino63_f16x3_input(const float* x, int64_t B, int64_t T, int64_t Cin, int64_t M, void* split_input,
+                                     size_t split_input_bytes, float* fbar, uint64_t* hot_slots, void* stream);
 
 
 int tspn_heads_f32(int mode, const float* a, const float* b, int64_t lda,
diff --git a/temporal-span-proposal-network-vidvrd_amd/_abi.py b/temporal-span-proposal-network-vidvrd_amd/_abi.py
--- a/temporal-span-proposal-network-vidvrd_amd/_abi.py
+++ b/temporal-span-proposal-network-vidvrd_amd/_abi.py
@@ -147,6 +147,9 @@
     "tspn_conv3_tc_wino63_f16x3_workspace_bytes": (_sz, [_i64, _i64, _i64, _i64]),
     "tspn_conv3_tc_wino63_f16x3": (_int, [_vp, _i64, _i64, _i64, _vp, _i64, _vp, _int, _vp, _vp, _sz, _vp]),
     "tspn_conv3_tc_wino63_f16x3_set_tail_split": (_int, [_int]),
+    "tspn_conv3_tc_wino63_f16x3_input_form": (_int, [_i64, _i64, _i64, _int]),
+    "tspn_conv3_tc_wino63_f16x3_set_input_form": (_int, [_int]),
+    "tspn_conv3_tc_wino63_f16x3_input": (_int, [_vp, _i64, _i64, _i64, _i64, _vp, _sz, _vp, _vp, _vp]),
     "tspn_span_predicate_workspace_bytes": (_sz, [_i64, _i64, _i64, _i64]),
     "tspn_span_predicate_f32": (_int, [_vp, _i64, _i64, _i64, _vp, _vp, _i64, _vp, _vp, _i64, _vp, _vp, _sz, _vp]),
     "tspn_decode_span_relations_workspace_bytes": (_sz, [_i64] * 8),
diff --git a/temporal-span-proposal-network-vidvrd_amd/build.py b/temporal-span-proposal-network-vidvrd_amd/build.py
--- a/temporal-span-proposal-network-vidvrd_amd/build.py
+++ b/temporal-span-proposal-network-vidvrd_amd/build.py
@@ -17,6 +17,7 @@
 CSRC_SPANLOSS = os.path.join(CSRC, "spanloss")
 CSRC_SPANSAMPLE = os.path.join(CSRC, "spansample")
 CSRC_PAIRLABELS = os.path.join(CSRC, "pairlabels")
+CSRC_INPUTF16 = os.path.join(CSRC, "inputf16")
 LIB_NAME = "libtspn_mi355x.so"
 LIB_PATH = os.path.join(HERE, LIB_NAME)
 ARCH = "gfx950"
@@ -43,7 +44,7 @@
                   glob.glob(os.path.join(CSRC_REL, "*.hip")) + glob.glob(os.path.join(CSRC_PAIRLIST, "*.hip")) +
                   glob.glob(os.path.join(CSRC_SPANBF16, "*.hip")) + glob.glob(os.path.join(CSRC_SPANLOSS, "*.hip")) +
                   glob.glob(os.path.join(CSRC_PAIRF16, "*.hip")) + glob.glob(os.path.join(CSRC_SPANSAMPLE, "*.hip")) +
-                  glob.glob(os.path.join(CSRC_PAIRLABELS, "*.hip")))
+                  glob.glob(os.path.join(CSRC_PAIRLABELS, "*.hip")) + glob.glob(os.path.join(CSRC_INPUTF16, "*.hip")))
 
 
 def _headers():
@@ -51,7 +52,7 @@
         glob.glob(os.path.join(CSRC_REL, "*.h")) + glob.glob(os.path.join(CSRC_PAIRLIST, "*.h")) + \
         glob.glob(os.path.join(CSRC_SPANBF16, "*.h")) + glob.glob(os.path.join(CSRC_SPANLOSS, "*.h")) + \
         glob.glob(os.path.join(CSRC_PAIRF16, "*.h")) + glob.glob(os.path.join(CSRC_SPANSAMPLE, "*.h")) + \
-        glob.glob(os.path.join(CSRC_PAIRLABELS, "*.h")) + \
+        glob.glob(os.path.join(CSRC_PAIRLABELS, "*.h")) + glob.glob(os.path.join(CSRC_INPUTF16, "*.h")) + \
         glob.glob(os.path.join(ROOT, "include", "*.h")) + \
         [os.path.abspath(__file__)]
 
diff --git a/temporal-span-proposal-network-vidvrd_amd/csrc/inputf16/tspn_input_f16x3.hip b/temporal-span-proposal-network-vidvrd_amd/csrc/inputf16/tspn_input_f16x3.hip
--- /dev/null
+++ b/temporal-span-proposal-network-vidvrd_amd/csrc/inputf16/tspn_input_f16x3.hip
@@ -0,0 +1,147 @@
+#include "tspn_common.h"
+#include "tspn_device.h"
+#include "tspn_wino63_input.h"
+
+namespace {
+
+using namespace tspn_dev;
+
+constexpr int IN_THREADS = 512;
+constexpr int IN_WAVES = IN_THREADS / 64;
+constexpr int NJ = 8;
+constexpr int SCAN_Q = 32;
+constexpr int PAD_SEXTETS = 64;
+
+__global__ __launch_bounds__(IN_THREADS) void input_f16x3_scan_kernel(
+    const float* __restrict__ x, int* __restrict__ Ve, float* __restrict__ fbar, int T, int Cin, int nq, int64_t NT,
+    int64_t nsext, int64_t nsp2, unsigned long long* __restrict__ hot) {
+  __shared__ float red[IN_WAVES][SCAN_Q * NJ];
+  const int tid = threadIdx.x, lane = tid & 63, wave = tid >> 6, nwaves = blockDim.x >> 6;
+
+  if ((int64_t)blockIdx.x >= NT) {
+    const int64_t S0 = nsext + (int64_t)(blockIdx.x - NT) * PAD_SEXTETS;
+    const int ns = (int)(nsp2 - S0 < PAD_SEXTETS ? nsp2 - S0 : PAD_SEXTETS);
+    for (int c = tid; c < NJ * ns; c += blockDim.x) Ve[(int64_t)(c / ns) * nsp2 + S0 + c % ns] = 0;
+    return;
+  }
+
+  const int64_t b = blockIdx.x;
+  const bool act = 4 * tid < Cin;
+  const int ch = act ? 4 * tid : 0;
+  float4 acc = make_float4(0.f, 0.f, 0.f, 0.f);
+  unsigned long long key = 0;
+  f32x4 d[8];
+  wino63_load_frames<2>(x, b, -1, T, Cin, act, ch, d + 6);
+  for (int q0 = 0; q0 < nq; q0 += SCAN_Q) {
+    const int nqc = nq - q0 < SCAN_Q ? nq - q0 : SCAN_Q;
+    for (int ql = 0; ql < nqc; ++ql) {
+      const int q = q0 + ql;
+      d[0] = d[6];
+      d[1] = d[7];
+      wino63_load_frames<6>(x, b, 6 * q + 1, T, Cin, act, ch, d + 2);
+      if (fbar != nullptr) {
+#pragma unroll
+        for (int k = 1; k <= 6; ++k)
+          if (6 * q + k - 1 < T) {
+            const f32x4 v = d[k];
+            acc.x += v.x; acc.y += v.y; acc.z += v.z; acc.w += v.w;
+          }
+      }
+      if (hot != nullptr) {
+        float m = 0.f;
+        wino63_absmax_own_frames(d, m);
+        const unsigned long long k = ((unsigned long long)__float_as_uint(m) << 32) | (unsigned)(b * nq + q);
+        key = k > key ? k : key;
+      }
+      f32x4 V[NJ];
+      wino63_bt(d, V);
+      float cm[NJ];
+#pragma unroll
+      for (int j = 0; j < NJ; ++j) {
+        float m = wino63_absmax4(0.f, V[j]);
+#pragma unroll
+        for (int o = 1; o < 64; o <<= 1) m = __builtin_elementwise_maximum(m, __shfl_xor(m, o, 64));
+        cm[j] = m;
+      }
+      if (lane == 0) {
+#pragma unroll
+        for (int j = 0; j < NJ; ++j) red[wave][ql * NJ + j] = cm[j];
+      }
+    }
+    __syncthreads();
+    for (int c = tid; c < nqc * NJ; c += blockDim.x) {
+      float m = red[0][c];
+      for (int w = 1; w < nwaves; ++w) m = __builtin_elementwise_maximum(m, red[w][c]);
+      Ve[(int64_t)(c & 7) * nsp2 + b * nq + q0 + (c >> 3)] = split_exponent((double)m);
+    }
+    __syncthreads();
+  }
+  if (hot != nullptr) wino63_hot_publish(hot, key, (unsigned)(blockIdx.x * IN_WAVES + wave));
+  if (fbar != nullptr && act) {
+    const float ft = (float)T;
+    *reinterpret_cast<float4*>(fbar + b * Cin + ch) = make_float4(acc.x / ft, acc.y / ft, acc.z / ft, acc.w / ft);
+  }
+}
+
+__global__ __launch_bounds__(256) void input_f16x3_split_kernel(
+    const float* __restrict__ x, const int* __restrict__ Ve, _Float16* __restrict__ Vh, int T, int Cin, int nq,
+    int64_t nsext, int64_t nsp2) {
+  const int tid = threadIdx.x, s = tid & 7, cg = blockIdx.y * 32 + (tid >> 3);
+  const int ncg = Cin >> 3;
+  if (cg >= ncg) return;
+  const int64_t S = (int64_t)blockIdx.x * 8 + s;
+  const bool ok = S < nsext;
+  const int64_t b = ok ? S / nq : 0;
+  const int q = ok ? (int)(S - b * nq) : 0;
+  int ecol[NJ];
+#pragma unroll
+  for (int j = 0; j < NJ; ++j) ecol[j] = Ve[(int64_t)j * nsp2 + S];
+  f32x4 V[2][NJ];
+#pragma unroll
+  for (int h = 0; h < 2; ++h) {
+    f32x4 d[8];
+    wino63_load_sextet(x, b, q, T, Cin, ok, 8 * cg + 4 * h, d);
+    wino63_bt(d, V[h]);
+  }
+#pragma unroll
+  for (int j = 0; j < NJ; ++j) {
+    f16x8 hi, lo;
+#pragma unroll
+    for (int i = 0; i < 8; ++i) {
+      _Float16 h, l;
+      wino63_split_f16(V[i >> 2][j][i & 3], ecol[j], h, l);
+      hi[i] = h;
+      lo[i] = l;
+    }
+    _Float16* dst = Vh + (((int64_t)j * 2 * ncg + cg) * nsp2 + S) * 8;
+    *reinterpret_cast<f16x8*>(dst) = hi;
+    *reinterpret_cast<f16x8*>(dst + (int64_t)ncg * nsp2 * 8) = lo;
+  }
+}
+
+}
+
+bool tspn::input_f16x3_supported(int64_t T, int64_t Cin) {
+  return T > 0 && Cin > 0 && Cin % 8 == 0 && Cin <= 4 * IN_THREADS;
+}
+
+int tspn::input_f16x3(const float* x, int64_t NT, int64_t T, int64_t Cin, int64_t nsp2, _Float16* Vh, int* Ve, float* fbar,
+                      uint64_t* hot, void* stream, int stages) {
+  const char* what = "tspn_conv3_tc_wino63_f16x3(fused input)";
+  TSPN_REQUIRE(NT > 0 && tspn::input_f16x3_supported(T, Cin), TSPN_EUNSUPPORTED, "%s: needs Cin %% 8 == 0, Cin <= %d (Cin=%lld)",
+               what, 4 * IN_THREADS, (long long)Cin);
+  TSPN_REQUIRE(x && Vh && Ve && tspn::all_aligned16(x, Vh, Ve, fbar), TSPN_EINVAL, "%s: null or unaligned pointer", what);
+  const int64_t nq = tspn::ceil_div(T, 6), nsext = NT * nq;
+  TSPN_REQUIRE(nsp2 >= nsext && nsp2 % 8 == 0, TSPN_EINVAL, "%s: %lld padded sextets for %lld", what, (long long)nsp2,
+               (long long)nsext);
+  const int64_t grid = NT + tspn::ceil_div(nsp2 - nsext, PAD_SEXTETS);
+  TSPN_REQUIRE(grid < (1LL << 31) && nsp2 / 8 < (1LL << 31), TSPN_EUNSUPPORTED, "%s: grid too large", what);
+  const int threads = (int)tspn::align_up((size_t)(Cin / 4), 64);
+  if (stages & TSPN_INPUT_SCAN)
+    hipLaunchKernelGGL(input_f16x3_scan_kernel, dim3((unsigned)grid), dim3(threads), 0, TSPN_STREAM(stream), x, Ve, fbar, (int)T,
+                       (int)Cin, (int)nq, NT, nsext, nsp2, reinterpret_cast<unsigned long long*>(hot));
+  if (stages & TSPN_INPUT_SPLIT)
+    hipLaunchKernelGGL(input_f16x3_split_kernel, dim3((unsigned)(nsp2 / 8), (unsigned)tspn::ceil_div(Cin / 8, 32)), dim3(256), 0,
+                       TSPN_STREAM(stream), x, Ve, Vh, (int)T, (int)Cin, (int)nq, nsext, nsp2);
+  return tspn::check_launch(what);
+}
diff --git a/temporal-span-proposal-network-vidvrd_amd/csrc/pairf16/tspn_heads_pair_f16x3.hip b/temporal-span-proposal-network-vidvrd_amd/csrc/pairf16/tspn_heads_pair_f16x3.hip
--- a/temporal-span-proposal-network-vidvrd_amd/csrc/pairf16/tspn_heads_pair_f16x3.hip
+++ b/temporal-span-proposal-network-vidvrd_amd/csrc/pairf16/tspn_heads_pair_f16x3.hip
@@ -32,12 +32,30 @@
   const int lane = threadIdx.x & 63, h = threadIdx.x >> 6;
   float mx = 0.f;
   bool finite = true;
-  if (h < H) {
-    for (int c = lane; c < C; c += 64) {
-      const float a = fabsf(Wh[(int64_t)h * C + c]);
-      finite = finite && (a < __builtin_inff());
-      mx = fmaxf(mx, a);
-    }
+  auto take = [&](float w, float& m) {
+    const float a = fabsf(w);
+    finite = finite && (a < __builtin_inff());
+    m = fmaxf(m, a);
+  };
+  if (h < H && (reinterpret_cast<uintptr_t>(Wh) & 15) == 0) {
+    const float4* row = reinterpret_cast<const float4*>(Wh + (int64_t)h * C);
+    const int n4 = C >> 2;
+    float m[4] = {0.f, 0.f, 0.f, 0.f};
+    int c = lane;
+    for (; c + 192 < n4; c += 256) {
+      float4 v[4];
+#pragma unroll
+      for (int u = 0; u < 4; ++u) v[u] = row[c + 64 * u];
+#pragma unroll
+      for (int u = 0; u < 4; ++u) { take(v[u].x, m[u]); take(v[u].y, m[u]); take(v[u].z, m[u]); take(v[u].w, m[u]); }
+    }
+    for (; c < n4; c += 64) {
+      const float4 v = row[c];
+      take(v.x, m[0]); take(v.y, m[0]); take(v.z, m[0]); take(v.w, m[0]);
+    }
+    mx = fmaxf(fmaxf(m[0], m[1]), fmaxf(m[2], m[3]));
+  } else if (h < H) {
+    for (int c = lane; c < C; c += 64) take(Wh[(int64_t)h * C + c], mx);
   }
 #pragma unroll
   for (int o = 32; o > 0; o >>= 1) mx = fmaxf(mx, __shfl_xor(mx, o, 64));
diff --git a/temporal-span-proposal-network-vidvrd_amd/csrc/tspn_common.h b/temporal-span-proposal-network-vidvrd_amd/csrc/tspn_common.h
--- a/temporal-span-proposal-network-vidvrd_amd/csrc/tspn_common.h
+++ b/temporal-span-proposal-network-vidvrd_amd/csrc/tspn_common.h
@@ -95,7 +95,13 @@
 bool wino63_f16x3_supported(int64_t Cin, int64_t M);
 size_t wino63_f16x3_workspace_bytes(int64_t B, int64_t T, int64_t Cin, int64_t M);
 int wino63_f16x3_input_transform(const float* x, int64_t B, int64_t T, int64_t Cin, int64_t M, void* workspace,
-                                 size_t workspace_bytes, void* stream, uint64_t* hot = nullptr);
+                                 size_t workspace_bytes, void* stream, uint64_t* hot = nullptr, bool fused_in = false,
+                                 float* fbar = nullptr, int stages = 3);
+bool wino63_f16x3_fused_input(int64_t B, int64_t T, int64_t Cin);
+constexpr int TSPN_INPUT_SCAN = 1, TSPN_INPUT_SPLIT = 2;
+bool input_f16x3_supported(int64_t T, int64_t Cin);
+int input_f16x3(const float* x, int64_t NT, int64_t T, int64_t Cin, int64_t nsp2, _Float16* Vh, int* Ve, float* fbar,
+                uint64_t* hot, void* stream, int stages = TSPN_INPUT_SCAN | TSPN_INPUT_SPLIT);
 int wino63_f16x3_contract(void* workspace, size_t workspace_bytes, int64_t B, int64_t T, int64_t Cin,
                           const int16_t* packed, int64_t M, const float* bias, int relu, float* y, int64_t ldy,
                           void* stream);
diff --git a/temporal-span-proposal-network-vidvrd_amd/csrc/tspn_fused.hip b/temporal-span-proposal-network-vidvrd_amd/csrc/tspn_fused.hip
--- a/temporal-span-proposal-network-vidvrd_amd/csrc/tspn_fused.hip
+++ b/temporal-span-proposal-network-vidvrd_amd/csrc/tspn_fused.hip
@@ -102,7 +102,19 @@
   if (e != hipSuccess)
     return tspn::fail(TSPN_ELAUNCH, "tspn_forward_fused: bias staging: %s", hipGetErrorString(e));
 
-  if ((rc = tspn_temporal_mean_f32(d->feats, NT, T, D, 1, fbar, stream))) return rc;
+  const bool guard = w63 && d->conv_check > 0 && d->conv_weight != nullptr;
+  uint64_t* hot = guard ? reinterpret_cast<uint64_t*>(ws + L.hot) : nullptr;
+  if (guard && hipMemsetAsync(hot, 0, TSPN_CONV_CHECK_SCRATCH_BYTES, s) != hipSuccess)
+    return tspn::fail(TSPN_ELAUNCH, "tspn_forward_fused: guard staging: %s", hipGetErrorString(hipGetLastError()));
+  uint64_t* hot_slots = hot ? hot + TSPN_CONV_CHECK_HOT_OFFSET / 8 : nullptr;
+
+  const bool fused_in = f16x3 && tspn::wino63_f16x3_fused_input(NT, T, D);
+  if (fused_in)
+    rc = tspn::wino63_f16x3_input_transform(d->feats, NT, T, D, 2 * C, ws + L.vt, L.vt_bytes, stream, hot_slots, true, fbar,
+                                            tspn::TSPN_INPUT_SCAN);
+  else
+    rc = tspn_temporal_mean_f32(d->feats, NT, T, D, 1, fbar, stream);
+  if (rc) return rc;
   (void)pooled;
   if ((rc = tspn::pair_predicate(fbar, NT, D, d->pairs, d->P, d->cls_w, d->cls_b, d->K, d->out_logits, lin,
                                  L.lin_bytes, stream)))
@@ -112,15 +124,12 @@
   const int64_t ldy =
       (tc && d->canonical_pairs && T % 2 == 0) ? (int64_t)tspn::align_up((size_t)T, 4) : T;
   if (!tc && (rc = tspn_transpose_td_f32(d->feats, NT, T, D, xt, stream))) return rc;
-  const bool guard = w63 && d->conv_check > 0 && d->conv_weight != nullptr;
-  uint64_t* hot = guard ? reinterpret_cast<uint64_t*>(ws + L.hot) : nullptr;
-  if (guard && hipMemsetAsync(hot, 0, TSPN_CONV_CHECK_SCRATCH_BYTES, s) != hipSuccess)
-    return tspn::fail(TSPN_ELAUNCH, "tspn_forward_fused: guard staging: %s", hipGetErrorString(hipGetLastError()));
-  uint64_t* hot_slots = hot ? hot + TSPN_CONV_CHECK_HOT_OFFSET / 8 : nullptr;
   if (f16x3) {
-    if ((rc = tspn::wino63_f16x3_input_transform(d->feats, NT, T, D, 2 * C, ws + L.vt, L.vt_bytes, stream, hot_slots)))
+    if ((rc = tspn::wino63_f16x3_input_transform(d->feats, NT, T, D, 2 * C, ws + L.vt, L.vt_bytes, stream, hot_slots, fused_in,
+                                                 nullptr, tspn::TSPN_INPUT_SPLIT)))
       return rc;
-  } else if (w63 && (rc = tspn::wino63_input_transform(d->feats, NT, T, D, ws + L.vt, L.vt_bytes, stream, hot_slots))) {
+  } else if (w63 && !f16x3 &&
+             (rc = tspn::wino63_input_transform(d->feats, NT, T, D, ws + L.vt, L.vt_bytes, stream, hot_slots))) {
     return rc;
   }
   if (d->ev_conv_begin) (void)hipEventRecord(static_cast<hipEvent_t>(d->ev_conv_begin), s);
diff --git a/temporal-span-proposal-network-vidvrd_amd/csrc/tspn_wino63.hip b/temporal-span-proposal-network-vidvrd_amd/csrc/tspn_wino63.hip
--- a/temporal-span-proposal-network-vidvrd_amd/csrc/tspn_wino63.hip
+++ b/temporal-span-proposal-network-vidvrd_amd/csrc/tspn_wino63.hip
@@ -4,6 +4,7 @@
 
 #include "tspn_common.h"
 #include "tspn_device.h"
+#include "tspn_wino63_input.h"
 
 namespace {
 
@@ -63,49 +64,6 @@
   }
 }
 
-__device__ __forceinline__ void wino63_load_sextet(const float* __restrict__ x, int64_t b, int q, int T, int Cin,
-                                                   int64_t ncols, bool ok, int channel_offset, f32x4 (&d)[8]) {
-#pragma unroll
-  for (int i = 0; i < 8; ++i) {
-    const int t = 6 * q + i - 1;
-    int64_t n = b * T + t;
-    n = n < 0 ? 0 : (n < ncols ? n : ncols - 1);
-    const f32x4 v = *reinterpret_cast<const f32x4*>(x + n * Cin + channel_offset);
-    d[i] = (ok && t >= 0 && t < T) ? v : f32x4{0.f, 0.f, 0.f, 0.f};
-  }
-}
-__device__ __forceinline__ void wino63_bt(const f32x4 (&d)[8], f32x4 (&V)[8]) {
-  V[0] = d[0] - d[6] + 5.25f * (d[4] - d[2]);
-  V[7] = d[7] - d[1] + 5.25f * (d[3] - d[5]);
-  {
-    const f32x4 t1 = d[2] + d[6] - 4.25f * d[4], t2 = d[1] + d[5] - 4.25f * d[3];
-    V[1] = t1 + t2;
-    V[2] = t1 - t2;
-  }
-  {
-    const f32x4 t1 = d[6] + 0.25f * d[2] - 1.25f * d[4], t2 = 0.5f * d[1] - 2.5f * d[3] + 2.f * d[5];
-    V[3] = t1 + t2;
-    V[4] = t1 - t2;
-  }
-  {
-    const f32x4 t1 = d[6] + 4.f * (d[2] - 1.25f * d[4]), t2 = 2.f * d[1] - 2.5f * d[3] + 0.5f * d[5];
-    V[5] = t1 + t2;
-    V[6] = t1 - t2;
-  }
-}
-__device__ __forceinline__ void wino63_absmax_own_frames(const f32x4 (&d)[8], float& m) {
-#pragma unroll
-  for (int i = 1; i < 7; ++i)
-    m = __builtin_elementwise_maximum(
-        __builtin_elementwise_maximum(m, __builtin_elementwise_maximum(fabsf(d[i][0]), fabsf(d[i][1]))),
-        __builtin_elementwise_maximum(fabsf(d[i][2]), fabsf(d[i][3])));
-}
-__device__ __forceinline__ void wino63_hot_publish(unsigned long long* __restrict__ hot, unsigned long long key, unsigned slot) {
-  key = tspn::wave_max_u64(key);
-  if ((threadIdx.x & 63) == 0)
-    __hip_atomic_fetch_max(hot + 32 * (slot & (TSPN_CONV_CHECK_HOT_SLOTS - 1)), key, __ATOMIC_RELAXED,
-                           __HIP_MEMORY_SCOPE_AGENT);
-}
 
 __global__ __launch_bounds__(256) void wino63_input_transform_kernel(
     const float* __restrict__ x, float* __restrict__ Vg, int T, int Cin, int nq, int64_t nsext, int64_t nsp,
@@ -119,7 +77,7 @@
   const int64_t b = ok ? S / nq : 0;
   const int q = ok ? (int)(S - b * nq) : 0;
   f32x4 d[8], V[8];
-  wino63_load_sextet(x, b, q, T, Cin, ncols, ok, 4 * cg, d);
+  wino63_load_sextet(x, b, q, T, Cin, ok, 4 * cg, d);
   if (hot) {
     float m = 0.f;
     wino63_absmax_own_frames(d, m);
@@ -357,13 +315,6 @@
 static_assert(TSPN_WINO63_GM > 0 && TSPN_WINO63_GM < 256, "the contraction's GM argument carries the tail split and the piece form above bit 7");
 constexpr size_t F_PARK_PER_TILE = (size_t)7 * F_THREADS * 128 * sizeof(float);
 
-__device__ __forceinline__ int split_exponent(double mx) {
-  if (!(mx > 0.0) || !(mx <= 1.7976931348623157e308)) return 0;
-  int k;
-  (void)frexp(mx, &k);
-  return 15 - k;
-}
-
 __device__ __forceinline__ double wino63_u(int j, double g0, double g1, double g2) {
   switch (j) {
     case 0: return g0;
@@ -424,7 +375,7 @@
 #pragma unroll
     for (int h = 0; h < 2; ++h) {
       f32x4 d[8];
-      wino63_load_sextet(x, b, q, T, Cin, ncols, ok, 8 * cg + 4 * h, d);
+      wino63_load_sextet(x, b, q, T, Cin, ok, 8 * cg + 4 * h, d);
       if (want_max) wino63_absmax_own_frames(d, xmax);
       wino63_bt(d, V[h]);
     }
@@ -440,9 +391,7 @@
     for (int j = 0; j < NJ; ++j)
 #pragma unroll
       for (int h = 0; h < 2; ++h)
-        cmax[j] = __builtin_elementwise_maximum(
-            __builtin_elementwise_maximum(cmax[j], __builtin_elementwise_maximum(fabsf(V[h][j][0]), fabsf(V[h][j][1]))),
-            __builtin_elementwise_maximum(fabsf(V[h][j][2]), fabsf(V[h][j][3])));
+        cmax[j] = wino63_absmax4(cmax[j], V[h][j]);
   }
   if (hot)
     wino63_hot_publish(hot, ((unsigned long long)__float_as_uint(xm) << 32) | (unsigned)(ok ? S : 0),
@@ -474,10 +423,10 @@
       f16x8 hi, lo;
 #pragma unroll
       for (int i = 0; i < 8; ++i) {
-        const float u = ldexpf(V[i >> 2][j][i & 3], ecol[j]);
-        const _Float16 h = (_Float16)u;
+        _Float16 h, l;
+        wino63_split_f16(V[i >> 2][j][i & 3], ecol[j], h, l);
         hi[i] = h;
-        lo[i] = (_Float16)(u - (float)h);
+        lo[i] = l;
       }
       _Float16* dst = Vh + (((int64_t)j * 2 * ncg + cg) * nsp2 + S) * 8;
       *reinterpret_cast<f16x8*>(dst) = hi;
@@ -934,7 +883,8 @@
 }
 
 int tspn::wino63_f16x3_input_transform(const float* x, int64_t B, int64_t T, int64_t Cin, int64_t M, void* workspace,
-                                       size_t workspace_bytes, void* stream, uint64_t* hot) {
+                                       size_t workspace_bytes, void* stream, uint64_t* hot, bool fused_in, float* fbar,
+                                       int stages) {
   const char* what = "tspn_conv3_tc_wino63_f16x3(input transform)";
   if (int rc = check_common(what, B, T, Cin, 32, T)) return rc;
   TSPN_REQUIRE(tspn::wino63_f16x3_supported(Cin, M), TSPN_EUNSUPPORTED,
@@ -950,6 +900,9 @@
   const int64_t nsext = B * nq, nsp2 = padded_sextets_f16x3(B, T);
   TSPN_REQUIRE(nsp2 / 8 < (1LL << 31), TSPN_EUNSUPPORTED, "%s: grid too large", what);
   char* ws = static_cast<char*>(workspace);
+  if (fused_in)
+    return tspn::input_f16x3(x, B, T, Cin, nsp2, reinterpret_cast<_Float16*>(ws + L.v), reinterpret_cast<int*>(ws + L.e), fbar,
+                             hot, stream, stages);
   void (*kern)(const float*, _Float16*, int*, int, int, int, int64_t, int64_t, int64_t, unsigned long long*) =
       wino63_input_transform_kernel;
   hipLaunchKernelGGL(kern, dim3((unsigned)(nsp2 / 8)), dim3(256), 0, TSPN_STREAM(stream), x,
@@ -975,6 +928,25 @@
   if (hipDeviceGetAttribute(&cus, hipDeviceAttributeMultiprocessorCount, dev) != hipSuccess || cus <= 0) return 0;
   if (tracked) cached[dev].store(cus, std::memory_order_relaxed);
   return cus;
+}
+
+extern "C" int tspn_conv3_tc_wino63_f16x3_input_form(int64_t NT, int64_t T, int64_t Cin, int cus) {
+  if (NT <= 0 || cus <= 0 || !tspn::input_f16x3_supported(T, Cin)) return 0;
+  return Cin >= 1024 && 2 * NT >= cus;
+}
+
+static std::atomic<int> g_input_form{0};
+
+extern "C" int tspn_conv3_tc_wino63_f16x3_set_input_form(int form) {
+  TSPN_REQUIRE(form >= 0 && form <= 2, TSPN_EINVAL, "tspn_conv3_tc_wino63_f16x3_set_input_form: form must be 0, 1 or 2");
+  return g_input_form.exchange(form, std::memory_order_relaxed);
+}
+
+bool tspn::wino63_f16x3_fused_input(int64_t B, int64_t T, int64_t Cin) {
+  const int form = g_input_form.load(std::memory_order_relaxed);
+  if (form == 1 || B <= 0) return false;
+  if (form == 2) return tspn::input_f16x3_supported(T, Cin);
+  return tspn_conv3_tc_wino63_f16x3_input_form(B, T, Cin, device_cus()) != 0;
 }
 
 static int tail_split_factor(int64_t tiles, int cus, int64_t* R) {
@@ -1036,6 +1008,19 @@
     TSPN_REQUIRE(tspn::aligned16(packed) && (reinterpret_cast<uintptr_t>(y) & 3) == 0,
                  TSPN_EUNSUPPORTED, "%s: packed weights must be 16-byte aligned", what);
   }
-  if (int rc = tspn::wino63_f16x3_input_transform(x, B, T, Cin, M, workspace, workspace_bytes, stream)) return rc;
+  if (int rc = tspn::wino63_f16x3_input_transform(x, B, T, Cin, M, workspace, workspace_bytes, stream, nullptr,
+                                                  tspn::wino63_f16x3_fused_input(B, T, Cin)))
+    return rc;
   return tspn::wino63_f16x3_contract(workspace, workspace_bytes, B, T, Cin, packed, M, bias, relu, y, T, stream);
 }
+
+extern "C" int tspn_conv3_tc_wino63_f16x3_input(const float* x, int64_t B, int64_t T, int64_t Cin, int64_t M, void* split_input,
+                                                size_t split_input_bytes, float* fbar, uint64_t* hot_slots, void* stream) {
+  const char* what = "tspn_conv3_tc_wino63_f16x3_input";
+  if (int rc = check_common(what, B, T, Cin, 32, T)) return rc;
+  const bool fused_in = tspn::wino63_f16x3_fused_input(B, T, Cin);
+  if (int rc = tspn::wino63_f16x3_input_transform(x, B, T, Cin, M, split_input, split_input_bytes, stream, hot_slots, fused_in, fbar))
+    return rc;
+  if (fbar != nullptr && !fused_in) return tspn_temporal_mean_f32(x, B, T, Cin, 1, fbar, stream);
+  return TSPN_OK;
+}
diff --git a/temporal-span-proposal-network-vidvrd_amd/csrc/tspn_wino63_input.h b/temporal-span-proposal-network-vidvrd_amd/csrc/tspn_wino63_input.h
--- /dev/null
+++ b/temporal-span-proposal-network-vidvrd_amd/csrc/tspn_wino63_input.h
@@ -0,0 +1,69 @@
+#pragma once
+#include "tspn_common.h"
+#include "tspn_device.h"
+
+namespace tspn_dev {
+
+template <int NF>
+__device__ __forceinline__ void wino63_load_frames(const float* __restrict__ x, int64_t b, int t0, int T, int Cin, bool ok,
+                                                   int channel_offset, f32x4* d) {
+#pragma unroll
+  for (int i = 0; i < NF; ++i) {
+    const int t = t0 + i;
+    const int64_t n = b * T + (t < 0 ? 0 : (t < T ? t : T - 1));
+    const f32x4 v = *reinterpret_cast<const f32x4*>(x + n * Cin + channel_offset);
+    d[i] = (ok && t >= 0 && t < T) ? v : f32x4{0.f, 0.f, 0.f, 0.f};
+  }
+}
+__device__ __forceinline__ void wino63_load_sextet(const float* __restrict__ x, int64_t b, int q, int T, int Cin, bool ok,
+                                                   int channel_offset, f32x4* d) {
+  wino63_load_frames<8>(x, b, 6 * q - 1, T, Cin, ok, channel_offset, d);
+}
+__device__ __forceinline__ void wino63_bt(const f32x4* d, f32x4 (&V)[8]) {
+  V[0] = d[0] - d[6] + 5.25f * (d[4] - d[2]);
+  V[7] = d[7] - d[1] + 5.25f * (d[3] - d[5]);
+  {
+    const f32x4 t1 = d[2] + d[6] - 4.25f * d[4], t2 = d[1] + d[5] - 4.25f * d[3];
+    V[1] = t1 + t2;
+    V[2] = t1 - t2;
+  }
+  {
+    const f32x4 t1 = d[6] + 0.25f * d[2] - 1.25f * d[4], t2 = 0.5f * d[1] - 2.5f * d[3] + 2.f * d[5];
+    V[3] = t1 + t2;
+    V[4] = t1 - t2;
+  }
+  {
+    const f32x4 t1 = d[6] + 4.f * (d[2] - 1.25f * d[4]), t2 = 2.f * d[1] - 2.5f * d[3] + 0.5f * d[5];
+    V[5] = t1 + t2;
+    V[6] = t1 - t2;
+  }
+}
+__device__ __forceinline__ float wino63_absmax4(float m, const f32x4 v) {
+  return __builtin_elementwise_maximum(
+      __builtin_elementwise_maximum(m, __builtin_elementwise_maximum(fabsf(v[0]), fabsf(v[1]))),
+      __builtin_elementwise_maximum(fabsf(v[2]), fabsf(v[3])));
+}
+__device__ __forceinline__ void wino63_absmax_own_frames(const f32x4* d, float& m) {
+#pragma unroll
+  for (int i = 1; i < 7; ++i) m = wino63_absmax4(m, d[i]);
+}
+__device__ __forceinline__ void wino63_hot_publish(unsigned long long* __restrict__ hot, unsigned long long key, unsigned slot) {
+  key = tspn::wave_max_u64(key);
+  if ((threadIdx.x & 63) == 0)
+    __hip_atomic_fetch_max(hot + 32 * (slot & (TSPN_CONV_CHECK_HOT_SLOTS - 1)), key, __ATOMIC_RELAXED,
+                           __HIP_MEMORY_SCOPE_AGENT);
+}
+
+__device__ __forceinline__ int split_exponent(double mx) {
+  if (!(mx > 0.0) || !(mx <= 1.7976931348623157e308)) return 0;
+  int k;
+  (void)frexp(mx, &k);
+  return 15 - k;
+}
+__device__ __forceinline__ void wino63_split_f16(float v, int e, _Float16& hi, _Float16& lo) {
+  const float u = ldexpf(v, e);
+  hi = (_Float16)u;
+  lo = (_Float16)(u - (float)hi);
+}
+
+}
diff --git a/temporal-span-proposal-network-vidvrd_amd/ops.py b/temporal-span-proposal-network-vidvrd_amd/ops.py
--- a/temporal-span-proposal-network-vidvrd_amd/ops.py
+++ b/temporal-span-proposal-network-vidvrd_amd/ops.py
@@ -17,6 +17,7 @@
     "temporal_mean_bf16", "forward_fused_bf16", "span_predicate",
     "pack_span_cls_bf16", "span_predicate_bf16", "decode_span_relations_bf16", "bottleneck_block_bf16", "bottleneck_block_proj_bf16", "bottleneck_block_res_bf16",
     "proposal_pair_filter", "gather_rows", "wino63_set_piece_form", "wino63_f16x3_set_tail_split", "conv3_spot_check",
+    "wino63_f16x3_set_input_form", "wino63_f16x3_input_form", "wino63_f16x3_input",
     "pack_conv2d", "pack_conv2d_frag", "conv2d_nhwc", "roi_align_nhwc", "pack_conv2d_frag_bf16", "conv2d_nhwc_bf16", "max_pool_nhwc", "pack_conv2d_frag_cin4", "conv2d_nhwc_cin4", "max_pool_nhwc_bf16", "pack_stem_bf16", "stem_conv_bf16", "stem_pool_bf16", "bottleneck_tail_bf16",
     "eval_traj_volume", "eval_viou", "eval_greedy_match",
     "status_words", "status_fault", "status_clear", "status_selftest",
@@ -468,6 +469,32 @@
 
 def wino63_f16x3_set_tail_split(on):
     return _toggle("tspn_conv3_tc_wino63_f16x3_set_tail_split", on)
+
+
+def wino63_f16x3_set_input_form(form):
+    return _toggle("tspn_conv3_tc_wino63_f16x3_set_input_form", form)
+
+
+def wino63_f16x3_input_form(NT, T, Cin, cus):
+    return int(_abi.lib().tspn_conv3_tc_wino63_f16x3_input_form(int(NT), int(T), int(Cin), int(cus)))
+
+
+def wino63_f16x3_input(x, M, workspace=None, mean=True, hot=True):
+    _dev(x, "x")
+    B, T, Cin = x.shape
+    l = _abi.lib()
+    need = l.tspn_conv3_tc_wino63_f16x3_workspace_bytes(B, T, Cin, M)
+    workspace = _workspace(workspace, need, x.device, "wino63_f16x3_input", sizes=True)
+    fbar = torch.empty((B, Cin), dtype=torch.float32, device=x.device) if mean else None
+    slots = torch.zeros((64, 32), dtype=torch.int64, device=x.device) if hot else None
+    _abi.check(l.tspn_conv3_tc_wino63_f16x3_input(_p(x), B, T, Cin, M, _p(workspace),
+                                                  workspace.numel() * workspace.element_size(), _p(fbar), _p(slots), _stream()))
+    nsp2 = -(-(B * (-(-T // 6))) // 256) * 256
+    vbytes = 8 * 2 * Cin * nsp2 * 2
+    v = workspace[:vbytes].view(torch.int16).view(8, 2, Cin // 8, nsp2, 8)
+    eoff = -(-vbytes // 256) * 256
+    e = workspace[eoff:eoff + 8 * nsp2 * 4].view(torch.int32).view(8, nsp2)
+    return v, e, fbar, (slots[:, 0].max() if hot else None)
 
 
 def heads(a, head_w, head_b, b=None, ia=None, ib=None, bias=None, channels=None, num_pairs=None):
```

Result: faster. 1.270 million (median of 6 runs) (+1.5%).
